# Crocodoctopus/zkstark

Hardware: AMD Instinct MI355X
Metric: field-elements/s through LDE+Merkle+FRI (full STARK-101 prover) (higher is better)
Workload: dtype u32 (mod 3*2^30+1) + SHA-256

## Files before the change

zkstark_amd/csrc/domain.hip:

```cpp
#include <chrono>
#include <cstdarg>
#include <cstdio>
#include <new>

#include "internal.hpp"

namespace zk {
namespace impl {

namespace {
thread_local std::string g_last_error;
}

int fail(int code, const char* fmt, ...) {
    char buf[512];
    va_list ap;
    va_start(ap, fmt);
    vsnprintf(buf, sizeof buf, fmt, ap);
    va_end(ap);
    g_last_error = buf;
    return code;
}
const char* last_error() { return g_last_error.c_str(); }

Plan make_plan(uint32_t log_m) {
    Plan p;
    uint32_t np = (log_m + kMaxRadixLog - 1) / kMaxRadixLog;
    if (np == 0) np = 1;
    uint32_t base = log_m / np, extra = log_m % np;
    p.nd = np;
    for (uint32_t d = 0; d < np; ++d) p.bits[d] = base + (d < extra ? 1 : 0);
    return p;
}

uint32_t pick_logC(uint32_t log_total, uint32_t logR) {
    uint32_t cols = log_total - logR, cap = ntt_pass_tile_log(log_total, logR) - logR;
    return cols < cap ? cols : cap;
}

int build_table(uint32_t root, uint32_t log_order, DevTable* t) {
    uint32_t lo_bits = (log_order + 1) / 2, hi_bits = log_order - lo_bits;
    std::vector<uint32_t> lo((size_t)1 << lo_bits), hi((size_t)1 << hi_bits);
    uint32_t acc = 1;
    for (size_t j = 0; j < lo.size(); ++j) { lo[j] = to_mont(acc); acc = mulmod(acc, root); }
    uint32_t step = powmod(root, (uint64_t)1 << lo_bits);
    acc = 1;
    for (size_t j = 0; j < hi.size(); ++j) { hi[j] = to_mont(acc); acc = mulmod(acc, step); }
    HIPCHK(hipMalloc(&t->lo, lo.size() * 4));
    HIPCHK(hipMalloc(&t->hi, hi.size() * 4));
    HIPCHK(hipMemcpy(t->lo, lo.data(), lo.size() * 4, hipMemcpyHostToDevice));
    HIPCHK(hipMemcpy(t->hi, hi.data(), hi.size() * 4, hipMemcpyHostToDevice));
    t->lo_bits = lo_bits;
    return ZK_OK;
}
void free_table(DevTable* t) {
    if (t->lo) (void)hipFree(t->lo);
    if (t->hi) (void)hipFree(t->hi);
    t->lo = t->hi = nullptr;
}

int run_dif(const uint32_t* src, uint32_t* data, uint32_t log_m, const Plan& pl, PowTable tw_inv, uint32_t L, uint32_t scale_mont, hipStream_t s, Profiler* prof,
            uint32_t batch, size_t src_stride, size_t data_stride) {
    uint32_t inner = log_m;
    for (uint32_t d = 0; d < pl.nd; ++d) {
        inner -= pl.bits[d];
        NttPassArgs a{};
        a.batch = batch; a.src_stride = d == 0 ? src_stride : data_stride; a.dst_stride = data_stride;
        a.src = d == 0 ? src : data; a.dst = data; a.log_total = log_m;
        a.logR = pl.bits[d]; a.logS = inner; a.logC = pick_logC(log_m, a.logR); a.tile_log = ntt_pass_tile_log(log_m, a.logR);
        a.L = L; a.tw = tw_inv; a.scale_mont = (inner == 0) ? scale_mont : 0;
        HIPCHK(launch_ntt_pass(a, NTT_DIF, s, prof));
    }
    return ZK_OK;
}
int run_dit(uint32_t* data, uint32_t log_m, const Plan& pl, PowTable tw, uint32_t L, hipStream_t s) {
    uint32_t inner = 0;
    for (int d = (int)pl.nd - 1; d >= 0; --d) {
        NttPassArgs a{};
        a.src = data; a.dst = data; a.log_total = log_m;
        a.logR = pl.bits[d]; a.logS = inner; a.logC = pick_logC(log_m, a.logR); a.tile_log = ntt_pass_tile_log(log_m, a.logR);
        a.L = L; a.tw = tw;
        HIPCHK(launch_ntt_pass(a, NTT_DIT, s));
        inner += pl.bits[d];
    }
    return ZK_OK;
}



void dom_free(zk_dom* d) {
    if (!d) return;
    free_table(&d->H); free_table(&d->Hinv); free_table(&d->W);
    if (d->d_inv_xm1) (void)hipFree(d->d_inv_xm1);
    delete d;
}

int dom_make(int device, uint32_t log_n, uint32_t log_b, uint32_t shift, bool fold_only, hipStream_t stream, zk_dom** out) {
    *out = nullptr;
    if (log_n < 1 || log_b > 5 || log_n + log_b > 30 || log_n + log_b < 1)
        return fail(ZK_ERR_INVALID, "domain: need 1 <= log_n, log_blowup <= 5, log_n + log_blowup <= 30 (got %u, %u)", log_n, log_b);
    if (shift == 0 || shift >= P) return fail(ZK_ERR_INVALID, "domain: shift must be a non-zero canonical residue");
    HIPCHK(hipSetDevice(device));
    zk_dom* d = new (std::nothrow) zk_dom();
    if (!d) return fail(ZK_ERR_NOMEM, "out of host memory");
    d->device = device;
    d->log_n = log_n; d->log_b = log_b; d->L = log_n + log_b;
    d->n = (size_t)1 << log_n; d->B = (size_t)1 << log_b; d->N = d->n << log_b;
    d->shift = shift;
    d->g = root_of_unity(log_n);
    d->h = root_of_unity(d->L);
    d->plan = make_plan(log_n);
    int rc;
    if ((rc = build_table(d->h, d->L, &d->H)) || (rc = build_table(invmod(d->h), d->L, &d->Hinv))) { dom_free(d); return rc; }
    uint32_t gm1 = invmod(d->g);
    d->shift_mont = to_mont(shift);
    d->gm1_mont = to_mont(gm1);
    d->gm2_mont = to_mont(mulmod(gm1, gm1));
    d->gm3_mont = to_mont(mulmod(mulmod(gm1, gm1), gm1));
    d->ninv_mont = to_mont(invmod((uint32_t)(d->n % P)));
    d->inv2_mont = to_mont(invmod(2));
    {
        const uint32_t inv2 = invmod(2);
        uint32_t wr = shift;
        for (uint32_t r = 0; r < d->L && r < 32; ++r) { d->fold_k[r] = mulmod(invmod(wr), inv2); wr = mulmod(wr, wr); }
        uint32_t xn = powmod(shift, d->n);
        const uint32_t hn = powmod(d->h, d->n);
        for (size_t r = 0; r < d->B; ++r) { const uint32_t den = sub(xn, 1); d->inv_den[r] = den ? invmod(den) : 0u; xn = mulmod(xn, hn); }
    }
    if (!fold_only) {
        if ((rc = build_table(shift, log_n, &d->W))) { dom_free(d); return rc; }
        if (powmod(shift, d->N) == 1) { dom_free(d); return fail(ZK_ERR_INVALID, "domain: shift lies in the evaluation subgroup"); }
        hipError_t e = hipMalloc((void**)&d->d_inv_xm1, d->N * 4);
        if (e != hipSuccess) { dom_free(d); return fail(ZK_ERR_NOMEM, "hipMalloc(%zu) failed", d->N * 4); }
        d->device_bytes += d->N * 4;
        e = launch_build_inv_xm1(d->d_inv_xm1, d->L, d->H.view(), d->shift_mont, stream);
        if (e == hipSuccess) e = hipStreamSynchronize(stream);
        if (e != hipSuccess) { dom_free(d); return fail(ZK_ERR_HIP, "inv_xm1 build failed: %s", hipGetErrorString(e)); }
    }
    *out = d;
    return ZK_OK;
}

int dom_lde(const zk_dom* d, const uint32_t* d_trace, uint32_t* d_coef, uint32_t* d_out, hipStream_t s, Profiler* prof, uint32_t batch) {
    const size_t ts = batch > 1 ? d->n : 0, cs = batch > 1 ? 2 * d->n : 0, os = batch > 1 ? d->N : 0;
    int rc = run_dif(d_trace, d_coef, d->log_n, d->plan, d->Hinv.view(), d->L, 0, s, prof, batch, ts, cs);
    if (rc) return rc;
    uint32_t* d_prep = d_coef + d->n;
    CoefPrepArgs pa{};
    pa.log_n = d->log_n; pa.log_b = d->log_b;
    pa.tw = d->H.view(); pa.wtab = d->W.view(); pa.ninv_mont = d->ninv_mont;
    pa.nd = d->plan.nd;
    for (uint32_t t = 0; t < d->plan.nd; ++t) pa.dig_bits[t] = d->plan.bits[t];
    uint32_t inner = d->log_b;
    for (int q = (int)d->plan.nd - 1; q >= 0; --q) {
        NttPassArgs a{};
        a.log_total = d->L; a.logR = d->plan.bits[q]; a.logS = inner; a.logC = pick_logC(d->L, a.logR); a.tile_log = ntt_pass_tile_log(d->L, a.logR);
        a.L = d->L; a.tw = d->H.view();
        a.dst = d_out;
        a.batch = batch; a.dst_stride = os; a.src_stride = os;
        if (q == (int)d->plan.nd - 1) {
            if (a.logC < d->log_b) a.logC = d->log_b;
            a.src_stride = cs;
            const bool fuse = ntt_fast_ok(a, NTT_DIT_LDE);
            if (fuse) {
                a.src = d_coef;
                a.prep = 1; a.prep_log_n = d->log_n; a.prep_log_b = d->log_b; a.prep_ninv_mont = d->ninv_mont;
                a.prep_nd = d->plan.nd; a.prep_wtab = d->W.view();
                for (uint32_t t = 0; t < d->plan.nd; ++t) a.prep_bits[t] = d->plan.bits[t];
            } else {
                HIPCHK(launch_coef_prepare(d_coef, d_prep, pa, s, prof, batch, cs, cs));
                a.src = d_prep;
            }
            HIPCHK(launch_ntt_pass(a, NTT_DIT_LDE, s, prof));
        } else {
            a.src = d_out;
            HIPCHK(launch_ntt_pass(a, NTT_DIT, s, prof));
        }
        inner += d->plan.bits[q];
    }
    return ZK_OK;
}

int compose_args(const zk_dom* d, const uint32_t* d_f, uint32_t* d_cp, uint32_t first, uint32_t last,
                 const uint32_t alpha_raw[3], ComposeArgs& a) {
    a = ComposeArgs{};
    a.f = d_f; a.inv_xm1 = d->d_inv_xm1; a.cp = d_cp;
    a.logN = d->L; a.log_b = d->log_b;
    a.htab = d->H.view();
    a.w_mont = d->shift_mont; a.gm1_mont = d->gm1_mont; a.gm2_mont = d->gm2_mont; a.gm3_mont = d->gm3_mont;
    a.first = first % P; a.last = last % P;
    uint32_t a0 = alpha_raw[0] % P, a1 = alpha_raw[1] % P, a2 = alpha_raw[2] % P;
    a.alpha0_mont = to_mont(a0);
    a.alpha1g2_mont = to_mont(mulmod(a1, mulmod(d->g, d->g)));
    for (size_t r = 0; r < d->B; ++r) {
        if (d->inv_den[r] == 0) return fail(ZK_ERR_INVALID, "compose: x^n = 1 on the domain");
        a.zz[r] = to_mont(to_mont(mulmod(a2, d->inv_den[r])));
    }
    return ZK_OK;
}
int dom_compose(const zk_dom* d, const uint32_t* d_f, uint32_t* d_cp, uint32_t first, uint32_t last,
                const uint32_t alpha_raw[3], hipStream_t s, Profiler* prof) {
    ComposeArgs a;
    int rc = compose_args(d, d_f, d_cp, first, last, alpha_raw, a);
    if (rc) return rc;
    HIPCHK(launch_compose(a, s, prof));
    return ZK_OK;
}

int fold_args(const zk_dom* d, const uint32_t* d_in, uint32_t* d_out, uint32_t log_m, uint32_t round, uint32_t beta_raw, FoldArgs& a) {
    if (log_m < 1 || log_m + round != d->L) return fail(ZK_ERR_INVALID, "fold: layer size 2^%u does not match round %u of a 2^%u domain", log_m, round, d->L);
    a = FoldArgs{};
    a.in = d_in; a.out = d_out; a.log_m = log_m; a.round = round;
    a.hinv = d->Hinv.view(); a.L = d->L;
    a.inv2_mont = d->inv2_mont;
    a.c_mont = to_mont(mulmod(beta_raw % P, d->fold_k[round]));
    return ZK_OK;
}
int dom_fold(const zk_dom* d, const uint32_t* d_in, uint32_t* d_out, uint32_t log_m, uint32_t round, uint32_t beta_raw,
             hipStream_t s, Profiler* prof) {
    FoldArgs a;
    int rc = fold_args(d, d_in, d_out, log_m, round, beta_raw, a);
    if (rc) return rc;
    HIPCHK(launch_fri_fold(a, s, prof));
    return ZK_OK;
}

int fold_multi_args(const zk_dom* d, const uint32_t* d_in, uint32_t* d_out, uint32_t log_m, uint32_t round, uint32_t steps, uint32_t beta_raw,
                    FoldMultiArgs& a) {
    if (steps < 1 || steps > 3) return fail(ZK_ERR_INVALID, "fold: steps must be 1..3 (got %u)", steps);
    if (log_m < steps || log_m + round != d->L)
        return fail(ZK_ERR_INVALID, "fold: layer size 2^%u does not match round %u + %u steps of a 2^%u domain", log_m, round, steps, d->L);
    a = FoldMultiArgs{};
    a.in = d_in; a.out = d_out; a.log_m = log_m; a.round = round; a.steps = steps;
    a.hinv = d->Hinv.view();
    a.scale_mont = to_mont(invmod(1u << steps));
    const uint32_t S = 1u << steps;
    const uint32_t om_inv = invmod(powmod(d->h, (uint64_t)d->N >> steps));
    uint32_t bk = beta_raw % P, ok = om_inv;
    for (uint32_t k = 0; k < steps; ++k) {
        const uint32_t base = mulmod(bk, mulmod(d->fold_k[round + k], 2));
        uint32_t tw = 1;
        for (uint32_t t = 0; t < (S >> (k + 1)); ++t) { a.c_mont[S - (S >> k) + t] = to_mont(mulmod(base, tw)); tw = mulmod(tw, ok); }
        bk = mulmod(bk, bk); ok = mulmod(ok, ok);
    }
    return ZK_OK;
}
int fold_multi_batch_args(const zk_dom* d, const uint32_t* d_in, uint32_t* d_out, uint32_t log_m, uint32_t round, uint32_t steps,
                          const uint32_t* d_beta_raw, uint32_t beta_stride, uint32_t* d_work, uint32_t batch, FoldMultiBatchArgs& a) {
    a = FoldMultiBatchArgs{};
    if (int rc = fold_multi_args(d, d_in, d_out, log_m, round, steps, 1u, a.a)) return rc;
    if (batch < 1 || ((uint64_t)batch << log_m) > ((uint64_t)1 << 32))
        return fail(ZK_ERR_INVALID, "fold: a batch of %u layers of 2^%u values does not fit 2^32 values", batch, log_m);
    a.beta_raw = d_beta_raw; a.beta_stride = beta_stride; a.cb = d_work; a.batch = batch;
    return ZK_OK;
}
int dom_fold_multi_batch(const zk_dom* d, const uint32_t* d_in, uint32_t* d_out, uint32_t log_m, uint32_t round, uint32_t steps,
                         const uint32_t* d_beta_raw, uint32_t beta_stride, uint32_t* d_work, uint32_t batch, hipStream_t s, Profiler* prof) {
    FoldMultiBatchArgs a;
    int rc = fold_multi_batch_args(d, d_in, d_out, log_m, round, steps, d_beta_raw, beta_stride, d_work, batch, a);
    if (rc) return rc;
    HIPCHK(launch_fri_fold_multi_batch(a, s, prof));
    return ZK_OK;
}
int dom_fold_multi(const zk_dom* d, const uint32_t* d_in, uint32_t* d_out, uint32_t log_m, uint32_t round, uint32_t steps, uint32_t beta_raw,
                   hipStream_t s, Profiler* prof) {
    if (steps == 1) return dom_fold(d, d_in, d_out, log_m, round, beta_raw, s, prof);
    FoldMultiArgs a;
    int rc = fold_multi_args(d, d_in, d_out, log_m, round, steps, beta_raw, a);
    if (rc) return rc;
    HIPCHK(launch_fri_fold_multi(a, s, prof));
    return ZK_OK;
}


int wait_flag(const uint32_t* flag, uint32_t want, hipStream_t stream, int (*poll)(void*), void* poll_user, double timeout_s) {
    auto t0 = std::chrono::steady_clock::now();
// ... 37 lines not shown
```

zkstark_amd/csrc/internal.hpp:

```cpp
#pragma once
#include <hip/hip_runtime.h>

#include <cstddef>
#include <cstring>
#include <string>
#include <vector>

#include "../../include/zkstark_amd.h"
#include "field.hpp"
#include "kernels.hpp"
#include "transcript.hpp"

struct zk_channel {
    zk::Channel ch;
};

namespace zk {
namespace impl {

int fail(int code, const char* fmt, ...);
const char* last_error();

#define HIPCHK(expr)                                                                          \
    do {                                                                                      \
// ... 9 lines not shown
template <> struct AbiMin<zk_shard_stats>     { static constexpr uint32_t v = 112;  static constexpr const char* name = "zk_shard_stats"; };
template <> struct AbiMin<zk_shard_plan_info> { static constexpr uint32_t v = 200;  static constexpr const char* name = "zk_shard_plan_info"; };
template <> struct AbiMin<zk_chain_probe>     { static constexpr uint32_t v = 48;   static constexpr const char* name = "zk_chain_probe"; };
template <class T> inline size_t abi_bytes(const T* p, const char* who) {
    static_assert(sizeof(T) >= AbiMin<T>::v && offsetof(T, struct_size) == 0, "a struct of the C ABI shrank or lost its size field");
    const uint32_t n = p->struct_size;
    if (n < AbiMin<T>::v || n > (1u << 16) || (n > AbiMin<T>::v && n < sizeof(T))) {
        fail(ZK_ERR_INVALID, "%s: %s.struct_size is %u; the caller sets it to sizeof(%s) before the call (ZK_STRUCT_INIT): at least %u bytes "
                             "(ABI version 6), %zu in this library (ABI version %u) -- was the caller compiled against another zkstark_amd.h?",
             who, AbiMin<T>::name, n, AbiMin<T>::name, AbiMin<T>::v, sizeof(T), (unsigned)ZK_ABI_VERSION);
        return 0;
    }
    return n < sizeof(T) ? n : sizeof(T);
}
template <class T> inline int abi_put(T* out, const T& src, const char* who) {
    const size_t k = abi_bytes(out, who);
    if (!k) return ZK_ERR_INVALID;
    memcpy(reinterpret_cast<char*>(out) + sizeof(uint32_t), reinterpret_cast<const char*>(&src) + sizeof(uint32_t), k - sizeof(uint32_t));
    return ZK_OK;
}
template <class T> inline int abi_get(const T* in, T* local, const char* who) {
    const size_t k = abi_bytes(in, who);
    if (!k) return ZK_ERR_INVALID;
    memset(static_cast<void*>(local), 0, sizeof(T));
    memcpy(static_cast<void*>(local), in, k);
    local->struct_size = (uint32_t)sizeof(T);
    return ZK_OK;
}

constexpr uint32_t kMaxQueries = 64;
constexpr uint32_t kHostTopSingle = 8;
constexpr uint32_t kMaxHostLog = 10;
constexpr size_t kMailValsOff = kMailDigests + ((size_t)8 << kMaxHostLog);
constexpr size_t kMailWords = kMailValsOff + ((size_t)2 << kMaxHostLog);
constexpr uint32_t kMaxRadixLog = 8;

inline int check_proof_size(const char* who, uint32_t log_n, uint32_t log_b, uint32_t log_extra = 0) {
    if (log_n < 2 || log_b < 1 || log_b > 5 || log_n + log_b + log_extra > 30)
        return fail(ZK_ERR_INVALID, "%s: need 2 <= log_n, 1 <= log_blowup <= 5, log_n + log_blowup%s <= 30 (got %u, %u)", who,
                    log_extra ? " + log_batch" : "", log_n, log_b);
    if (log_n == 3)
        return fail(ZK_ERR_INVALID, "%s: n = 8 is degenerate for the Fibonacci-square constraints (the degree asserts of prover.rs:156/:169 would fail)", who);
    return ZK_OK;
}

struct Plan {
    uint32_t nd = 0;
    uint32_t bits[kMaxDigits] = {0};
};
Plan make_plan(uint32_t log_m);
uint32_t pick_logC(uint32_t log_total, uint32_t logR);

struct DevTable {
    uint32_t* lo = nullptr;
    uint32_t* hi = nullptr;
    uint32_t lo_bits = 0;
    PowTable view() const { return PowTable{lo, hi, lo_bits}; }
};
int build_table(uint32_t root, uint32_t log_order, DevTable* t);
void free_table(DevTable* t);

int run_dif(const uint32_t* src, uint32_t* data, uint32_t log_m, const Plan& pl, PowTable tw_inv, uint32_t L, uint32_t scale_mont,
            hipStream_t s, Profiler* prof = nullptr, uint32_t batch = 1, size_t src_stride = 0, size_t data_stride = 0);
int run_dit(uint32_t* data, uint32_t log_m, const Plan& pl, PowTable tw, uint32_t L, hipStream_t s);

constexpr uint32_t kGrindHostMaxBits = 10;
struct Grinder;
int grinder_create(int device, void* stream, uint32_t max_jobs, Grinder** out);
void grinder_destroy(Grinder* g);
int grind_device(Grinder* g, const uint8_t* states, size_t count, uint32_t bits, uint64_t start, uint64_t* nonces_out);
int grind_host(const uint8_t state[32], uint32_t bits, uint64_t start, uint32_t threads, uint64_t* nonce_out);
int grind_channel(Grinder* g, Channel& ch, uint32_t bits, uint64_t* nonce_out);

}
}

struct zk_dom {
    int device = 0;
    uint32_t log_n = 0, log_b = 0, L = 0;
    size_t n = 0, N = 0, B = 0;
    uint32_t shift = 0, g = 0, h = 0;
    zk::impl::DevTable H, Hinv, W;
    uint32_t* d_inv_xm1 = nullptr;
    zk::impl::Plan plan;
    uint32_t shift_mont = 0, gm1_mont = 0, gm2_mont = 0, gm3_mont = 0, ninv_mont = 0, inv2_mont = 0;
    uint32_t fold_k[32] = {0};
    uint32_t inv_den[32] = {0};
    size_t device_bytes = 0;
};

namespace zk {
namespace impl {

void dom_free(zk_dom* d);
int dom_make(int device, uint32_t log_n, uint32_t log_b, uint32_t shift, bool fold_only, hipStream_t stream, zk_dom** out);
int dom_lde(const zk_dom* d, const uint32_t* d_trace, uint32_t* d_coef, uint32_t* d_out, hipStream_t s, Profiler* prof, uint32_t batch = 1);
int compose_args(const zk_dom* d, const uint32_t* d_f, uint32_t* d_cp, uint32_t first, uint32_t last, const uint32_t alpha_raw[3], ComposeArgs& a);
int dom_compose(const zk_dom* d, const uint32_t* d_f, uint32_t* d_cp, uint32_t first, uint32_t last, const uint32_t alpha_raw[3],
                hipStream_t s, Profiler* prof);
int fold_args(const zk_dom* d, const uint32_t* d_in, uint32_t* d_out, uint32_t log_m, uint32_t round, uint32_t beta_raw, FoldArgs& a);
int dom_fold(const zk_dom* d, const uint32_t* d_in, uint32_t* d_out, uint32_t log_m, uint32_t round, uint32_t beta_raw, hipStream_t s,
             Profiler* prof);
int fold_multi_args(const zk_dom* d, const uint32_t* d_in, uint32_t* d_out, uint32_t log_m, uint32_t round, uint32_t steps, uint32_t beta_raw,
                    FoldMultiArgs& a);
int dom_fold_multi(const zk_dom* d, const uint32_t* d_in, uint32_t* d_out, uint32_t log_m, uint32_t round, uint32_t steps, uint32_t beta_raw,
                   hipStream_t s, Profiler* prof = nullptr);
int fold_multi_batch_args(const zk_dom* d, const uint32_t* d_in, uint32_t* d_out, uint32_t log_m, uint32_t round, uint32_t steps,
                          const uint32_t* d_beta_raw, uint32_t beta_stride, uint32_t* d_work, uint32_t batch, FoldMultiBatchArgs& a);
int dom_fold_multi_batch(const zk_dom* d, const uint32_t* d_in, uint32_t* d_out, uint32_t log_m, uint32_t round, uint32_t steps,
                         const uint32_t* d_beta_raw, uint32_t beta_stride, uint32_t* d_work, uint32_t batch, hipStream_t s,
                         Profiler* prof = nullptr);

int wait_flag(const uint32_t* flag, uint32_t want, hipStream_t stream, int (*poll)(void*) = nullptr, void* poll_user = nullptr, double timeout_s = 30.0);
double now_us();
int tail_open_begin(zk_ctx* tail, size_t x);
int tail_open_end(zk_ctx* tail, uint32_t* vals_out, uint8_t* paths_out);
void path_nodes(size_t m, size_t leaf, std::vector<size_t>& out);
int merkle_nodes_to_host(int device, hipStream_t s, const uint32_t* d_heap, size_t first, size_t count, uint8_t* out);

}
}
```

zkstark_amd/csrc/kernels.hip:

```cpp
#include "kernels.hpp"

#include <cstdlib>

#include "field.hpp"
#include "fieldhash_f64.hpp"
#include "sha256_quad.hpp"
#include "sha256.hpp"

namespace zk {

__device__ __forceinline__ uint32_t pow_lookup(const PowTable& t, uint32_t e) {
    return mont_mul(t.hi[e >> t.lo_bits], t.lo[e & ((1u << t.lo_bits) - 1u)]);
}

constexpr uint32_t R2_MONT = R2;

__device__ uint32_t mont_inv(uint32_t a) {
    uint32_t r = R1, b = a;
    uint32_t e = P - 2;
#pragma unroll 1
    for (int i = 0; i < 32; ++i) {
        if (e & 1) r = mont_mul(r, b);
        b = mont_mul(b, b);
        e >>= 1;
// ... 29 lines not shown
    const uint32_t col0 = blockIdx.x << logC;
    const uint32_t tile_elems = R << logC;
    const uint32_t tw_shift = p.L - logR - logS;
    const uint32_t smask = (1u << logS) - 1u;

    for (uint32_t j = tid; j < (R >> 1); j += kNttThreads) twl[j] = pow_lookup(p.tw, j << (p.L - logR));

    if (MODE == NTT_DIT_LDE) {
        const uint32_t logB = logS;
        const uint32_t a0 = col0 >> logB;
        for (uint32_t u = tid; u < (tile_elems >> logB); u += kNttThreads) {
            uint32_t ao = u >> logR, t = u & (R - 1u);
            uint32_t v = p.src[((size_t)(a0 + ao) << logR) | t];
            uint32_t row = __brev(t) >> (32u - logR);
            uint32_t* dstp = &tile[row * pitch + (ao << logB)];
            dstp[0] = v;
            for (uint32_t s = 1; s <= smask; ++s) dstp[s] = mont_mul(v, pow_lookup(p.tw, (t * s) << tw_shift));
        }
    } else {
        for (uint32_t l = tid; l < tile_elems; l += kNttThreads) {
            uint32_t t, c;
            tile_coords(l, logR, logS, logC, t, c);
            uint32_t col = col0 + c, a = col >> logS, s = col & smask;
            size_t addr = ((size_t)a << (logR + logS)) | ((size_t)t << logS) | s;
            uint32_t v = p.src[addr];
            uint32_t row = t;
            if (MODE == NTT_DIT) {
                if (logS) v = mont_mul(v, pow_lookup(p.tw, (t * s) << tw_shift));
                row = __brev(t) >> (32u - logR);
            }
            tile[row * pitch + c] = v;
        }
    }
    __syncthreads();

    const uint32_t nb = tile_elems >> 1;
    if (MODE == NTT_DIF) {
        for (int ll = (int)logR - 1; ll >= 0; --ll) {
            for (uint32_t b = tid; b < nb; b += kNttThreads) {
                uint32_t c = b & (C - 1u), pi = b >> logC;
                uint32_t j = pi & ((1u << ll) - 1u);
                uint32_t i = ((pi >> ll) << (ll + 1)) | j;
                uint32_t* x0 = &tile[i * pitch + c];
                uint32_t* x1 = x0 + (pitch << ll);
                uint32_t u = *x0, v = *x1;
                *x0 = add(u, v);
                *x1 = mont_mul(sub(u, v), twl[j << (logR - 1u - ll)]);
            }
            __syncthreads();
        }
    } else {
        for (uint32_t ll = 0; ll < logR; ++ll) {
            for (uint32_t b = tid; b < nb; b += kNttThreads) {
                uint32_t c = b & (C - 1u), pi = b >> logC;
                uint32_t j = pi & ((1u << ll) - 1u);
                uint32_t i = ((pi >> ll) << (ll + 1)) | j;
                uint32_t* x0 = &tile[i * pitch + c];
                uint32_t* x1 = x0 + (pitch << ll);
                uint32_t u = *x0, v = mont_mul(*x1, twl[j << (logR - 1u - ll)]);
                *x0 = add(u, v);
                *x1 = sub(u, v);
            }
            __syncthreads();
        }
    }

    for (uint32_t l = tid; l < tile_elems; l += kNttThreads) {
        uint32_t t, c;
        tile_coords(l, logR, logS, logC, t, c);
        uint32_t col = col0 + c, a = col >> logS, s = col & smask;
        size_t addr = ((size_t)a << (logR + logS)) | ((size_t)t << logS) | s;
        uint32_t v;
        if (MODE == NTT_DIF) {
            v = tile[(__brev(t) >> (32u - logR)) * pitch + c];
            if (logS) v = mont_mul(v, pow_lookup(p.tw, (t * s) << tw_shift));
            else if (p.scale_mont) v = mont_mul(v, p.scale_mont);
        } else {
            v = tile[t * pitch + c];
        }
        p.dst[addr] = v;
    }
}

bool launch_ntt_pass_fast(const NttPassArgs& a, NttMode mode, hipStream_t s, hipError_t* err);

hipError_t launch_ntt_pass(const NttPassArgs& a, NttMode mode, hipStream_t s, Profiler* prof) {
    double bytes = mode == NTT_DIT_LDE ? 4.0 * ((double)((size_t)1 << (a.log_total - a.logS)) + (double)((size_t)1 << a.log_total))
                                       : 8.0 * (double)((size_t)1 << a.log_total);
    const uint32_t batch = a.batch ? a.batch : 1;
    ScopedKernelTimer tm(prof, K_NTT, bytes * batch, s, kNttOpsPerElement * (double)((size_t)1 << a.log_total) * batch * (double)a.logR / 7.0);
    hipError_t ferr = hipSuccess;
    if (launch_ntt_pass_fast(a, mode, s, &ferr)) return ferr;
    uint32_t cols_log = a.log_total - a.logR;
    uint32_t blocks = 1u << (cols_log - a.logC);
    size_t shmem = ((size_t)(1u << a.logR) * ((1u << a.logC) + 1u) + (1u << a.logR) / 2u) * sizeof(uint32_t);
    switch (mode) {
        case NTT_DIF: hipLaunchKernelGGL(ntt_pass_kernel<NTT_DIF>, dim3(blocks, batch), dim3(kNttThreads), shmem, s, a); break;
        case NTT_DIT: hipLaunchKernelGGL(ntt_pass_kernel<NTT_DIT>, dim3(blocks, batch), dim3(kNttThreads), shmem, s, a); break;
        case NTT_DIT_LDE: hipLaunchKernelGGL(ntt_pass_kernel<NTT_DIT_LDE>, dim3(blocks, batch), dim3(kNttThreads), shmem, s, a); break;
    }
    return hipGetLastError();
}

__global__ __launch_bounds__(256) void coef_prepare_kernel(const uint32_t* U, uint32_t* out, CoefPrepArgs a, size_t u_stride, size_t out_stride) {
    const uint32_t pos = blockIdx.x * blockDim.x + threadIdx.x, n = 1u << a.log_n;
    if (pos >= n) return;
    U += (size_t)blockIdx.y * u_stride;
    out += (size_t)blockIdx.y * out_stride;
    uint32_t k = 0, rem = a.log_n, sh = 0;
    for (uint32_t d = 0; d < a.nd; ++d) {
        rem -= a.dig_bits[d];
        k |= ((pos >> rem) & ((1u << a.dig_bits[d]) - 1u)) << sh;
        sh += a.dig_bits[d];
    }
    const uint32_t c_top = U[n - 1u];
    uint32_t v = sub(U[pos], mont_mul(c_top, pow_lookup(a.tw, ((k + 1u) & (n - 1u)) << a.log_b)));
    out[pos] = mont_mul(v, mont_mul(pow_lookup(a.wtab, k), a.ninv_mont));
}

hipError_t launch_coef_prepare(const uint32_t* U, uint32_t* out, const CoefPrepArgs& a, hipStream_t s, Profiler* prof,
                               uint32_t batch, size_t u_stride, size_t out_stride) {
    uint32_t n = 1u << a.log_n;
    ScopedKernelTimer tm(prof, K_NTT, 8.0 * n * batch, s);
    hipLaunchKernelGGL(coef_prepare_kernel, dim3((n + 255) / 256, batch), dim3(256), 0, s, U, out, a, u_stride, out_stride);
    return hipGetLastError();
}

struct DigitArgs {
    uint32_t nd;
    uint32_t bits[kMaxDigits];
};

__global__ void digit_reverse_kernel(const uint32_t* in, uint32_t* out, uint32_t log_m, DigitArgs dg, int to_natural) {
    size_t pos = (size_t)blockIdx.x * blockDim.x + threadIdx.x;
    if (pos >= ((size_t)1 << log_m)) return;
    uint32_t k = 0, rem = log_m, sh = 0;
    for (uint32_t d = 0; d < dg.nd; ++d) {
        rem -= dg.bits[d];
        k |= (((uint32_t)pos >> rem) & ((1u << dg.bits[d]) - 1u)) << sh;
        sh += dg.bits[d];
    }
    if (to_natural) out[k] = in[pos];
    else out[pos] = in[k];
}

hipError_t launch_digit_reverse(const uint32_t* in, uint32_t* out, uint32_t log_m, uint32_t nd,
                                const uint32_t* dig_bits, int to_natural, hipStream_t s) {
    DigitArgs dg{};
    dg.nd = nd;
    for (uint32_t i = 0; i < nd; ++i) dg.bits[i] = dig_bits[i];
    size_t m = (size_t)1 << log_m;
    uint32_t threads = 256, blocks = (uint32_t)((m + threads - 1) / threads);
    hipLaunchKernelGGL(digit_reverse_kernel, dim3(blocks), dim3(threads), 0, s, in, out, log_m, dg, to_natural);
    return hipGetLastError();
}

__global__ void degree_check_kernel(const uint32_t* coef, uint32_t log_m, DigitArgs dg, uint32_t bound, uint32_t* out) {
    size_t pos = (size_t)blockIdx.x * blockDim.x + threadIdx.x;
    if (pos >= ((size_t)1 << log_m)) return;
    uint32_t k = 0, rem = log_m, sh = 0;
    for (uint32_t d = 0; d < dg.nd; ++d) {
        rem -= dg.bits[d];
        k |= (((uint32_t)pos >> rem) & ((1u << dg.bits[d]) - 1u)) << sh;
        sh += dg.bits[d];
    }
    const uint32_t v = coef[pos];
    if (k >= bound && v != 0) atomicAdd(&out[0], 1u);
    if (k + 1 == bound) out[1] = v;
}
hipError_t launch_degree_check(const uint32_t* coef, uint32_t log_m, uint32_t nd, const uint32_t* dig_bits, uint32_t bound, uint32_t* out, hipStream_t s) {
    DigitArgs dg{};
    dg.nd = nd;
    for (uint32_t i = 0; i < nd; ++i) dg.bits[i] = dig_bits[i];
    size_t m = (size_t)1 << log_m;
    hipLaunchKernelGGL(degree_check_kernel, dim3((uint32_t)((m + 255) / 256)), dim3(256), 0, s, coef, log_m, dg, bound, out);
    return hipGetLastError();
}


constexpr int kInvBatch = 8;

__global__ __launch_bounds__(256) void build_inv_xm1_kernel(uint32_t* out, size_t count, uint32_t e0, uint32_t order_mask, PowTable htab, uint32_t w_mont) {
    size_t gid = (size_t)blockIdx.x * blockDim.x + threadIdx.x;
    size_t base = gid * kInvBatch;
    if (base >= count) return;
    uint32_t d[kInvBatch], pre[kInvBatch];
    uint32_t acc = R1;
#pragma unroll
    for (int e = 0; e < kInvBatch; ++e) {
        size_t i = base + e;
        uint32_t x = i < count ? mont_mul(pow_lookup(htab, (e0 + (uint32_t)i) & order_mask), w_mont) : add(R1, R1);
        d[e] = sub(x, R1);
        pre[e] = acc;
        acc = mont_mul(acc, d[e]);
    }
    uint32_t inv = mont_inv(acc);
#pragma unroll
    for (int e = kInvBatch - 1; e >= 0; --e) {
        size_t i = base + e;
        uint32_t r = mont_mul(inv, pre[e]);
        inv = mont_mul(inv, d[e]);
        if (i < count) out[i] = r;
    }
}

hipError_t launch_build_inv_xm1_range(uint32_t* out, size_t count, uint32_t e0, uint32_t log_order, PowTable htab, uint32_t shift_mont, hipStream_t s) {
    size_t threads_total = (count + kInvBatch - 1) / kInvBatch;
    uint32_t blocks = (uint32_t)((threads_total + 255) / 256);
    if (!blocks) return hipSuccess;
    hipLaunchKernelGGL(build_inv_xm1_kernel, dim3(blocks), dim3(256), 0, s, out, count, e0, (uint32_t)(((uint64_t)1 << log_order) - 1u), htab, shift_mont);
    return hipGetLastError();
}
hipError_t launch_build_inv_xm1(uint32_t* out, uint32_t logN, PowTable htab, uint32_t shift_mont, hipStream_t s) {
    return launch_build_inv_xm1_range(out, (size_t)1 << logN, 0u, logN, htab, shift_mont, s);
}

struct ComposeRaw { uint32_t f0, f1, f2, inv0, inv2, x_hi, x_lo, zz; };
__device__ __forceinline__ ComposeRaw compose_fetch(const ComposeArgs& a, const uint32_t* f, size_t i) {
    const size_t N = (size_t)1 << a.logN;
    const uint32_t B = 1u << a.log_b;
    const size_t i1 = (i + B) & (N - 1), i2 = (i + 2 * (size_t)B) & (N - 1);
    ComposeRaw r;
    r.f0 = f[i]; r.f1 = f[i1]; r.f2 = f[i2];
    r.inv0 = a.inv_xm1[i]; r.inv2 = a.inv_xm1[i2];
    r.x_hi = a.htab.hi[(uint32_t)i >> a.htab.lo_bits]; r.x_lo = a.htab.lo[(uint32_t)i & ((1u << a.htab.lo_bits) - 1u)];
    r.zz = a.zz[i & (B - 1)];
    return r;
}
template <bool BATCH>
__device__ __forceinline__ uint32_t compose_eval(const ComposeArgs& a, uint32_t f0, uint32_t f1, uint32_t f2, uint32_t inv0, uint32_t inv2,
                                                 uint32_t x, uint32_t zz, uint32_t first, uint32_t last, uint32_t al0, uint32_t al1g2, uint32_t al2) {
    uint32_t t0 = mont_mul(mont_mul(sub(f0, first), inv0), al0);
    uint32_t t1 = mont_mul(mont_mul(sub(f0, last), inv2), al1g2);
    uint32_t v3 = mont_mul(mont_mul(sub(x, a.gm3_mont), sub(x, a.gm2_mont)), sub(x, a.gm1_mont));
    uint32_t y = mont_mul(v3, zz);
    if (BATCH) y = mont_mul(y, al2);
    uint32_t num = sub(sub(mont_mul(f2, 1u), mont_mul(f1, f1)), mont_mul(f0, f0));
    uint32_t t2 = mont_mul(num, y);
    return add(add(t0, t1), t2);
}
template <bool BATCH>
__device__ __forceinline__ uint32_t compose_finish(const ComposeArgs& a, const ComposeRaw& r, uint32_t first, uint32_t last, uint32_t al0,
                                                   uint32_t al1g2, uint32_t al2) {
    const uint32_t x = mont_mul(mont_mul(r.x_hi, r.x_lo), a.w_mont);
    return compose_eval<BATCH>(a, r.f0, r.f1, r.f2, r.inv0, r.inv2, x, r.zz, first, last, al0, al1g2, al2);
}
template <bool BATCH>
__device__ __forceinline__ uint32_t compose_core(const ComposeArgs& a, const uint32_t* f, uint32_t first, uint32_t last, uint32_t al0,
                                                 uint32_t al1g2, uint32_t al2, size_t i) {
    return compose_finish<BATCH>(a, compose_fetch(a, f, i), first, last, al0, al1g2, al2);
}
__device__ __forceinline__ uint32_t compose_at(const ComposeArgs& a, size_t i) {
    return compose_core<false>(a, a.f, a.first, a.last, a.alpha0_mont, a.alpha1g2_mont, 0u, i);
}

__global__ __launch_bounds__(256) void compose_kernel(ComposeArgs a) {
    size_t i = (size_t)blockIdx.x * blockDim.x + threadIdx.x;
    if (i >= ((size_t)1 << a.logN)) return;
    a.cp[i] = compose_at(a, i);
}

__global__ __launch_bounds__(256) void compose_kernel4(ComposeArgs a) {
    const size_t N = (size_t)1 << a.logN;
    const uint32_t B = 1u << a.log_b;
    const size_t i = ((size_t)blockIdx.x * blockDim.x + threadIdx.x) * 4;
    if (i >= N) return;
    const uint4* fv = reinterpret_cast<const uint4*>(a.f);
    const uint4* iv = reinterpret_cast<const uint4*>(a.inv_xm1);
    uint32_t f0[4], f1[4], f2[4], inv0[4], inv2[4], zz[4];
    const uint4 v0 = fv[i >> 2], w0 = iv[i >> 2];
    f0[0] = v0.x; f0[1] = v0.y; f0[2] = v0.z; f0[3] = v0.w;
    inv0[0] = w0.x; inv0[1] = w0.y; inv0[2] = w0.z; inv0[3] = w0.w;
    if (B >= 4) {
        const uint4 v1 = fv[((i + B) & (N - 1)) >> 2], v2 = fv[((i + 2 * (size_t)B) & (N - 1)) >> 2], w2 = iv[((i + 2 * (size_t)B) & (N - 1)) >> 2];
        f1[0] = v1.x; f1[1] = v1.y; f1[2] = v1.z; f1[3] = v1.w;
        f2[0] = v2.x; f2[1] = v2.y; f2[2] = v2.z; f2[3] = v2.w;
        inv2[0] = w2.x; inv2[1] = w2.y; inv2[2] = w2.z; inv2[3] = w2.w;
        const uint32_t z0 = (uint32_t)i & (B - 1);
#pragma unroll
        for (int k = 0; k < 4; ++k) zz[k] = a.zz[z0 + k];
    } else {
        const uint4 v1 = fv[((i + 4) & (N - 1)) >> 2], w1 = iv[((i + 4) & (N - 1)) >> 2];
        const uint32_t fw[8] = {v0.x, v0.y, v0.z, v0.w, v1.x, v1.y, v1.z, v1.w};
        const uint32_t iw[8] = {w0.x, w0.y, w0.z, w0.w, w1.x, w1.y, w1.z, w1.w};
#pragma unroll
        for (int k = 0; k < 4; ++k) {
            f1[k] = B == 1 ? fw[k + 1] : fw[k + 2];
            f2[k] = B == 1 ? fw[k + 2] : fw[k + 4];
            inv2[k] = B == 1 ? iw[k + 2] : iw[k + 4];
            zz[k] = B == 1 ? a.zz[0] : a.zz[k & 1];
        }
    }
    uint32_t x = mont_mul(pow_lookup(a.htab, (uint32_t)i), a.w_mont);
    const uint32_t h = pow_lookup(a.htab, 1u);
    uint32_t r[4];
#pragma unroll
    for (int k = 0; k < 4; ++k) {
        r[k] = compose_eval<false>(a, f0[k], f1[k], f2[k], inv0[k], inv2[k], x, zz[k], a.first, a.last, a.alpha0_mont, a.alpha1g2_mont, 0u);
        if (k < 3) x = mont_mul(x, h);
    }
    reinterpret_cast<uint4*>(a.cp)[i >> 2] = make_uint4(r[0], r[1], r[2], r[3]);
}

hipError_t launch_compose(const ComposeArgs& a, hipStream_t s, Profiler* prof) {
    size_t N = (size_t)1 << a.logN;
    ScopedKernelTimer tm(prof, K_COMPOSE, 8.0 * (double)N, s);
    const bool aligned = ((reinterpret_cast<uintptr_t>(a.f) | reinterpret_cast<uintptr_t>(a.inv_xm1) | reinterpret_cast<uintptr_t>(a.cp)) & 15u) == 0;
    if (a.logN >= 4 && aligned) {
        uint32_t blocks = (uint32_t)((N / 4 + 255) / 256);
        hipLaunchKernelGGL(compose_kernel4, dim3(blocks), dim3(256), 0, s, a);
    } else {
        uint32_t blocks = (uint32_t)((N + 255) / 256);
        hipLaunchKernelGGL(compose_kernel, dim3(blocks), dim3(256), 0, s, a);
    }
    return hipGetLastError();
}

struct FoldRaw { uint32_t u, v, x_hi, x_lo; };
__device__ __forceinline__ FoldRaw fold_fetch(const FoldArgs& a, size_t i) {
    const size_t half = (size_t)1 << (a.log_m - 1);
    const uint32_t e = (uint32_t)(i << a.round);
    FoldRaw r;
    r.u = a.in[i]; r.v = a.in[i + half];
    r.x_hi = a.hinv.hi[e >> a.hinv.lo_bits]; r.x_lo = a.hinv.lo[e & ((1u << a.hinv.lo_bits) - 1u)];
    return r;
}
__device__ __forceinline__ uint32_t fold_finish(const FoldArgs& a, const FoldRaw& r) {
    uint32_t xinv = mont_mul(r.x_hi, r.x_lo);
    uint32_t s = mont_mul(add(r.u, r.v), a.inv2_mont);
    uint32_t d = mont_mul(mont_mul(sub(r.u, r.v), xinv), a.c_mont);
    return add(s, d);
}
__device__ __forceinline__ uint32_t fold_at(const FoldArgs& a, size_t i) { return fold_finish(a, fold_fetch(a, i)); }

__global__ __launch_bounds__(256) void fri_fold_kernel(FoldArgs a) {
    size_t i = (size_t)blockIdx.x * blockDim.x + threadIdx.x;
    if (i >= ((size_t)1 << (a.log_m - 1))) return;
    a.out[i] = fold_at(a, i);
}

__global__ __launch_bounds__(256) void fri_fold_kernel4(FoldArgs a) {
    const size_t half = (size_t)1 << (a.log_m - 1);
    const size_t i = ((size_t)blockIdx.x * blockDim.x + threadIdx.x) * 4;
    if (i >= half) return;
    const uint4 u = reinterpret_cast<const uint4*>(a.in)[i >> 2], v = reinterpret_cast<const uint4*>(a.in)[(i + half) >> 2];
    const uint32_t uu[4] = {u.x, u.y, u.z, u.w}, vv[4] = {v.x, v.y, v.z, v.w};
    uint32_t xinv = pow_lookup(a.hinv, (uint32_t)(i << a.round));
    const uint32_t step = pow_lookup(a.hinv, 1u << a.round);
    uint32_t r[4];
#pragma unroll
    for (int k = 0; k < 4; ++k) {
        const uint32_t sm = mont_mul(add(uu[k], vv[k]), a.inv2_mont);
        const uint32_t d = mont_mul(mont_mul(sub(uu[k], vv[k]), xinv), a.c_mont);
        r[k] = add(sm, d);
        if (k < 3) xinv = mont_mul(xinv, step);
    }
    reinterpret_cast<uint4*>(a.out)[i >> 2] = make_uint4(r[0], r[1], r[2], r[3]);
}

hipError_t launch_fri_fold(const FoldArgs& a, hipStream_t s, Profiler* prof) {
    size_t half = (size_t)1 << (a.log_m - 1);
    ScopedKernelTimer tm(prof, K_FOLD, 12.0 * (double)half, s);
    const bool aligned = ((reinterpret_cast<uintptr_t>(a.in) | reinterpret_cast<uintptr_t>(a.out)) & 15u) == 0;
    if (half >= 4 && aligned) {
        uint32_t blocks = (uint32_t)((half / 4 + 255) / 256);
        hipLaunchKernelGGL(fri_fold_kernel4, dim3(blocks), dim3(256), 0, s, a);
    } else {
        uint32_t blocks = (uint32_t)((half + 255) / 256);
        hipLaunchKernelGGL(fri_fold_kernel, dim3(blocks), dim3(256), 0, s, a);
    }
    return hipGetLastError();
}

template <int STEPS>
__device__ __forceinline__ uint32_t fold_multi_core(const uint32_t (&c)[7], uint32_t scale_mont, uint32_t (&v)[1 << STEPS], uint32_t xinv) {
    constexpr int S = 1 << STEPS;
#pragma unroll
    for (int k = 0; k < STEPS; ++k) {
        const int cnt = S >> (k + 1);
#pragma unroll
        for (int t = 0; t < cnt; ++t) {
            const uint32_t u = v[t], w = v[t + cnt];
            v[t] = add(add(u, w), mont_mul(sub(u, w), mont_mul(xinv, c[S - (S >> k) + t])));
        }
        if (k + 1 < STEPS) xinv = mont_mul(xinv, xinv);
    }
    return mont_mul(v[0], scale_mont);
}
template <int STEPS>
__device__ __forceinline__ uint32_t fold_multi_one(const FoldMultiArgs& a, uint32_t (&v)[1 << STEPS], uint32_t xinv) {
    return fold_multi_core<STEPS>(a.c_mont, a.scale_mont, v, xinv);
}

template <int STEPS>
__global__ __launch_bounds__(256) void fri_fold_multi_kernel1(FoldMultiArgs a) {
    constexpr int S = 1 << STEPS;
    const size_t q = (size_t)1 << (a.log_m - STEPS);
    const size_t i = (size_t)blockIdx.x * blockDim.x + threadIdx.x;
    if (i >= q) return;
    uint32_t v[S];
#pragma unroll
    for (int t = 0; t < S; ++t) v[t] = a.in[i + t * q];
    a.out[i] = fold_multi_one<STEPS>(a, v, pow_lookup(a.hinv, (uint32_t)(i << a.round)));
}

template <int STEPS>
__global__ __launch_bounds__(256) void fri_fold_multi_kernel(FoldMultiArgs a) {
    constexpr int S = 1 << STEPS;
    const size_t q = (size_t)1 << (a.log_m - STEPS);
    const size_t i = ((size_t)blockIdx.x * blockDim.x + threadIdx.x) * 4;
    if (i >= q) return;
    uint4 ld[S];
#pragma unroll
    for (int t = 0; t < S; ++t) ld[t] = reinterpret_cast<const uint4*>(a.in)[(i + t * q) >> 2];
    uint32_t xinv = pow_lookup(a.hinv, (uint32_t)(i << a.round));
    const uint32_t step = pow_lookup(a.hinv, 1u << a.round);
    uint32_t r[4];
#pragma unroll
    for (int e = 0; e < 4; ++e) {
        uint32_t v[S];
#pragma unroll
        for (int t = 0; t < S; ++t) v[t] = e == 0 ? ld[t].x : e == 1 ? ld[t].y : e == 2 ? ld[t].z : ld[t].w;
        r[e] = fold_multi_one<STEPS>(a, v, xinv);
        if (e < 3) xinv = mont_mul(xinv, step);
    }
    reinterpret_cast<uint4*>(a.out)[i >> 2] = make_uint4(r[0], r[1], r[2], r[3]);
}

template <int STEPS>
static void fold_multi_launch(const FoldMultiArgs& a, size_t q, bool wide, hipStream_t s) {
    if (wide) hipLaunchKernelGGL(fri_fold_multi_kernel<STEPS>, dim3((uint32_t)((q / 4 + 255) / 256)), dim3(256), 0, s, a);
    else hipLaunchKernelGGL(fri_fold_multi_kernel1<STEPS>, dim3((uint32_t)((q + 255) / 256)), dim3(256), 0, s, a);
}
hipError_t launch_fri_fold_multi(const FoldMultiArgs& a, hipStream_t s, Profiler* prof) {
    if (a.steps < 1 || a.steps > 3 || a.log_m < a.steps) return hipErrorInvalidValue;
    const size_t m = (size_t)1 << a.log_m, q = m >> a.steps;
    ScopedKernelTimer tm(prof, K_FOLD, 4.0 * (double)(m + q), s);
    const bool wide = q >= 4 && ((reinterpret_cast<uintptr_t>(a.in) | reinterpret_cast<uintptr_t>(a.out)) & 15u) == 0;
    if (a.steps == 1) fold_multi_launch<1>(a, q, wide, s);
    else if (a.steps == 2) fold_multi_launch<2>(a, q, wide, s);
    else fold_multi_launch<3>(a, q, wide, s);
    return hipGetLastError();
}

template <int STEPS>
__global__ __launch_bounds__(256) void fri_fold_multi_batch_prep_kernel(FoldMultiBatchArgs p) {
    constexpr int S = 1 << STEPS;
    const uint32_t b = blockIdx.x * blockDim.x + threadIdx.x;
    if (b >= p.batch) return;
    uint32_t bk = mont_mul(p.beta_raw[(size_t)b * p.beta_stride], R2_MONT);
    uint32_t c[8] = {0, 0, 0, 0, 0, 0, 0, 0};
#pragma unroll
    for (int k = 0; k < STEPS; ++k) {
#pragma unroll
        for (int t = 0; t < (S >> (k + 1)); ++t) c[S - (S >> k) + t] = mont_mul(bk, p.a.c_mont[S - (S >> k) + t]);
        if (k + 1 < STEPS) bk = mont_mul(bk, bk);
    }
    uint32_t* row = p.cb + (size_t)b * 8;
#pragma unroll
    for (int j = 0; j < 8; ++j) row[j] = c[j];
}
template <int STEPS>
__device__ __forceinline__ void fold_multi_batch_consts(const FoldMultiBatchArgs& p, size_t b, uint32_t (&c)[7]) {
    constexpr int S = 1 << STEPS;
    const uint32_t* row = p.cb + b * 8;
#pragma unroll
    for (int j = 0; j < 7; ++j) c[j] = j < S - 1 ? row[j] : 0u;
}

template <int STEPS>
__global__ __launch_bounds__(256) void fri_fold_multi_batch_kernel1(FoldMultiBatchArgs p) {
    constexpr int S = 1 << STEPS;
    const uint32_t log_q = p.a.log_m - STEPS;
    const size_t q = (size_t)1 << log_q;
    const size_t pos = (size_t)blockIdx.x * blockDim.x + threadIdx.x;
    if (pos >= ((size_t)p.batch << log_q)) return;
    const size_t b = pos >> log_q, i = pos & (q - 1);
    const uint32_t* in = p.a.in + (b << p.a.log_m);
    uint32_t v[S];
#pragma unroll
    for (int t = 0; t < S; ++t) v[t] = in[i + t * q];
    uint32_t c[7];
    fold_multi_batch_consts<STEPS>(p, b, c);
    p.a.out[pos] = fold_multi_core<STEPS>(c, p.a.scale_mont, v, pow_lookup(p.a.hinv, (uint32_t)(i << p.a.round)));
}

template <int STEPS>
__global__ __launch_bounds__(256) void fri_fold_multi_batch_kernel(FoldMultiBatchArgs p) {
    constexpr int S = 1 << STEPS;
    const uint32_t log_q = p.a.log_m - STEPS;
    const size_t q = (size_t)1 << log_q;
    const size_t pos = ((size_t)blockIdx.x * blockDim.x + threadIdx.x) * 4;
    if (pos >= ((size_t)p.batch << log_q)) return;
    const size_t b = pos >> log_q, i = pos & (q - 1);
    const uint32_t* in = p.a.in + (b << p.a.log_m);
    uint4 ld[S];
#pragma unroll
    for (int t = 0; t < S; ++t) ld[t] = reinterpret_cast<const uint4*>(in)[(i + t * q) >> 2];
    uint32_t c[7];
    fold_multi_batch_consts<STEPS>(p, b, c);
    uint32_t xinv = pow_lookup(p.a.hinv, (uint32_t)(i << p.a.round));
    const uint32_t step = pow_lookup(p.a.hinv, 1u << p.a.round);
    uint32_t r[4];
#pragma unroll
    for (int e = 0; e < 4; ++e) {
        uint32_t v[S];
#pragma unroll
        for (int t = 0; t < S; ++t) v[t] = e == 0 ? ld[t].x : e == 1 ? ld[t].y : e == 2 ? ld[t].z : ld[t].w;
        r[e] = fold_multi_core<STEPS>(c, p.a.scale_mont, v, xinv);
        if (e < 3) xinv = mont_mul(xinv, step);
    }
    reinterpret_cast<uint4*>(p.a.out)[pos >> 2] = make_uint4(r[0], r[1], r[2], r[3]);
}

template <int STEPS>
static void fold_multi_batch_launch(const FoldMultiBatchArgs& p, size_t total, bool wide, hipStream_t s) {
    hipLaunchKernelGGL(fri_fold_multi_batch_prep_kernel<STEPS>, dim3((p.batch + 255) / 256), dim3(256), 0, s, p);
    if (wide) hipLaunchKernelGGL(fri_fold_multi_batch_kernel<STEPS>, dim3((uint32_t)((total / 4 + 255) / 256)), dim3(256), 0, s, p);
    else hipLaunchKernelGGL(fri_fold_multi_batch_kernel1<STEPS>, dim3((uint32_t)((total + 255) / 256)), dim3(256), 0, s, p);
}
hipError_t launch_fri_fold_multi_batch(const FoldMultiBatchArgs& p, hipStream_t s, Profiler* prof) {
    const FoldMultiArgs& a = p.a;
    if (a.steps < 1 || a.steps > 3 || a.log_m < a.steps || a.log_m > 32 || p.batch < 1 || !p.beta_raw || !p.cb) return hipErrorInvalidValue;
    const size_t m = (size_t)1 << a.log_m, q = m >> a.steps, total = (size_t)p.batch * q;
    if ((size_t)p.batch * m > ((size_t)1 << 32)) return hipErrorInvalidValue;
    ScopedKernelTimer tm(prof, K_FOLD, 4.0 * (double)p.batch * (double)(m + q), s);
    const bool wide = q >= 4 && ((reinterpret_cast<uintptr_t>(a.in) | reinterpret_cast<uintptr_t>(a.out)) & 15u) == 0;
    if (a.steps == 1) fold_multi_batch_launch<1>(p, total, wide, s);
    else if (a.steps == 2) fold_multi_batch_launch<2>(p, total, wide, s);
    else fold_multi_batch_launch<3>(p, total, wide, s);
    return hipGetLastError();
}


__constant__ FieldHashConsts g_fh_consts;
__constant__ FieldHashConsts64 g_fh_consts64;

template <int HASH> struct Hasher;
template <> struct Hasher<0> {
    static __device__ __forceinline__ Digest leaf(uint32_t v) { return sha256_leaf(v); }
    static __device__ __forceinline__ Digest inner(const Digest& l, const Digest& r) { return sha256_inner(l, r); }
};
template <> struct Hasher<1> {
    static __device__ __forceinline__ Digest leaf(uint32_t v) { return fieldhash_leaf64(v, g_fh_consts64); }
    static __device__ __forceinline__ Digest inner(const Digest& l, const Digest& r) { return fieldhash_inner64(l, r, g_fh_consts64); }
};

struct PlainSrc {
    const uint32_t* vals;
    using Raw = uint32_t;
    __device__ __forceinline__ Raw fetch(size_t pos) const { return vals[pos]; }
    __device__ __forceinline__ uint32_t finish(const Raw& r, size_t) const { return r; }
    __device__ __forceinline__ uint32_t load(size_t pos) const { return vals[pos]; }
};
struct FoldSrc {
    FoldArgs a;
    using Raw = FoldRaw;
    __device__ __forceinline__ void prepare() { if (a.dyn) a.c_mont = *a.dyn; }
    __device__ __forceinline__ Raw fetch(size_t pos) const { return fold_fetch(a, pos); }
    __device__ __forceinline__ uint32_t finish(const Raw& r, size_t pos) const { uint32_t v = fold_finish(a, r); a.out[pos] = v; return v; }
    __device__ __forceinline__ uint32_t load(size_t pos) const { return finish(fetch(pos), pos); }
};
struct ComposeSrc {
    ComposeArgs a;
    using Raw = size_t;
    __device__ __forceinline__ Raw fetch(size_t pos) const { return pos; }
    __device__ __forceinline__ uint32_t finish(const Raw& r, size_t) const { return load(r); }
    __device__ __forceinline__ uint32_t load(size_t pos) const { uint32_t v = compose_at(a, pos); a.cp[pos] = v; return v; }
};

struct ComposeBlockSrc {
    ComposeBlockArgs b;
    using Raw = size_t;
    __device__ __forceinline__ uint32_t f_at(size_t t) const {
        const uint32_t gmask = (1u << b.lg) - 1u;
        if (t >> b.log_m) {
            const size_t v = t - ((size_t)1 << b.log_m);
            return b.halo[(v & gmask) * b.halo_stride + (v >> b.lg)];
        }
        const uint32_t log_cl = b.lg + b.log_cnt;
        const size_t piece = ((t >> log_cl) << b.lg) | (t & gmask);
        return b.a.f[(piece << b.log_cnt) | ((t & (((size_t)1 << log_cl) - 1)) >> b.lg)];
    }
    __device__ __forceinline__ Raw fetch(size_t pos) const { return pos; }
    __device__ __forceinline__ uint32_t finish(const Raw& r, size_t) const { return load(r); }
    __device__ __forceinline__ uint32_t load(size_t pos) const {
        const ComposeArgs& a = b.a;
        const size_t B = (size_t)1 << a.log_b;
        const uint32_t f0 = f_at(pos), f1 = f_at(pos + B), f2 = f_at(pos + 2 * B);
        const uint32_t x = mont_mul(pow_lookup(a.htab, b.e0 + (uint32_t)pos), a.w_mont);
        return compose_eval<false>(a, f0, f1, f2, a.inv_xm1[pos], a.inv_xm1[pos + 2 * B], x, a.zz[pos & (B - 1)], a.first, a.last, a.alpha0_mont,
                                   a.alpha1g2_mont, 0u);
    }
};

struct ComposeBatchSrc {
    ComposeArgs a;
    const BatchChal* chal;
    using Raw = size_t;
    __device__ __forceinline__ Raw fetch(size_t pos) const { return pos; }
    __device__ __forceinline__ uint32_t finish(const Raw& r, size_t) const { return load(r); }
    __device__ __forceinline__ uint32_t load(size_t pos) const {
        const size_t b = pos >> a.logN, i = pos & (((size_t)1 << a.logN) - 1);
        const BatchChal c = chal[b];
        uint32_t v = compose_core<true>(a, a.f + (b << a.logN), c.first, c.last, c.alpha0_mont, c.alpha1g2_mont, c.alpha2_mont, i);
        a.cp[pos] = v;
        return v;
    }
};
struct FoldBatchSrc {
    FoldArgs a;
    const BatchChal* chal;
    using Raw = size_t;
    __device__ __forceinline__ Raw fetch(size_t pos) const { return pos; }
    __device__ __forceinline__ uint32_t finish(const Raw& r, size_t) const { return load(r); }
    __device__ __forceinline__ uint32_t load(size_t pos) const {
        const uint32_t lh = a.log_m - 1;
        const size_t half = (size_t)1 << lh, b = pos >> lh, i = pos & (half - 1);
        const uint32_t* in = a.in + (b << a.log_m);
        uint32_t u = in[i], v = in[i + half];
        uint32_t xinv = pow_lookup(a.hinv, (uint32_t)(i << a.round));
        uint32_t s = mont_mul(add(u, v), a.inv2_mont);
        uint32_t d = mont_mul(mont_mul(sub(u, v), xinv), chal[b].c_mont);
        uint32_t r = add(s, d);
        a.out[pos] = r;
        return r;
    }
};

struct InterleaveSrc {
    const uint32_t* recv;
    uint32_t log_parts, log_cnt;
    using Raw = uint32_t;
    __device__ __forceinline__ uint32_t load(size_t pos) const {
        return recv[((pos & (((size_t)1 << log_parts) - 1)) << log_cnt) | (pos >> log_parts)];
    }
    __device__ __forceinline__ Raw fetch(size_t pos) const { return load(pos); }
    __device__ __forceinline__ uint32_t finish(const Raw& r, size_t) const { return r; }
};

template <class S> __device__ __forceinline__ auto src_prepare(S& s, int) -> decltype(s.prepare(), void()) { s.prepare(); }
template <class S> __device__ __forceinline__ void src_prepare(S&, long) {}

constexpr int kMerkleThreads = 256;
constexpr uint32_t kMerkleMaxK = 4;

__device__ __forceinline__ void store_digest(uint32_t* nodes, size_t node, const Digest& d) {
    uint4* q = reinterpret_cast<uint4*>(nodes + node * 8);
    q[0] = make_uint4(d.w[0], d.w[1], d.w[2], d.w[3]);
    q[1] = make_uint4(d.w[4], d.w[5], d.w[6], d.w[7]);
}
__device__ __forceinline__ Digest load_digest(const uint32_t* nodes, size_t node) {
    const uint4* q = reinterpret_cast<const uint4*>(nodes + node * 8);
    uint4 lo = q[0], hi = q[1];
    Digest d;
    d.w[0] = lo.x; d.w[1] = lo.y; d.w[2] = lo.z; d.w[3] = lo.w;
    d.w[4] = hi.x; d.w[5] = hi.y; d.w[6] = hi.z; d.w[7] = hi.w;
    return d;
}

__device__ __forceinline__ Digest lds_digest(const uint4* p) {
    uint4 lo = p[0], hi = p[1];
    Digest d;
    d.w[0] = lo.x; d.w[1] = lo.y; d.w[2] = lo.z; d.w[3] = lo.w;
    d.w[4] = hi.x; d.w[5] = hi.y; d.w[6] = hi.z; d.w[7] = hi.w;
    return d;
}

template <class SRC, bool LEAF, int HASH>
__global__ __launch_bounds__(kMerkleThreads) void merkle_subtree_kernel(SRC src, uint32_t* nodes,
                                                                        uint32_t depth_in, uint32_t k, size_t off) {
    extern __shared__ __attribute__((aligned(16))) uint4 stage[];
    src_prepare(src, 0);
    const uint32_t lane = threadIdx.x & 63u, wave = threadIdx.x >> 6;
    const size_t gwave = (size_t)blockIdx.x * (kMerkleThreads / 64) + wave;
    const size_t base = (gwave << (6 + k)) + off;
    const size_t in_base = ((size_t)1 << depth_in) - 1;
    uint4* my = stage + (size_t)wave * (k + 1) * 128;
    uint4* scratch = my + (size_t)k * 128;
    typename SRC::Raw raw;
    Digest dnext;
    uint32_t val = 0;
    if (LEAF) val = src.load(base + lane - off);
    else dnext = load_digest(nodes, in_base + base + lane);
#pragma unroll 1
    for (uint32_t i = 0; i < (1u << k); ++i) {
        Digest d;
        const size_t pos = base + (size_t)i * 64 + lane;
        const bool more = i + 1 < (1u << k);
        if (LEAF) {
            if (more) raw = src.fetch(pos + 64 - off);
            d = Hasher<HASH>::leaf(val);
            store_digest(nodes, in_base + pos, d);
        } else {
            d = dnext;
            if (more) dnext = load_digest(nodes, in_base + pos + 64);
        }
        uint32_t idx = i, lvl = 0;
#pragma unroll 1
        while (lvl < k) {
            uint4* left = my + lvl * 128;
            uint4* grp = (idx & 1u) ? scratch : left;
            grp[2 * lane] = make_uint4(d.w[0], d.w[1], d.w[2], d.w[3]);
            grp[2 * lane + 1] = make_uint4(d.w[4], d.w[5], d.w[6], d.w[7]);
            if (!(idx & 1u)) break;
// ... 387 lines not shown
    static bool done[64] = {false};
    int dev = 0;
    hipError_t e = hipGetDevice(&dev);
    if (e != hipSuccess) return e;
    if (dev < 0 || dev >= 64 || done[dev]) return hipSuccess;
    FieldHashConsts c;
    fieldhash_make_consts(c);
    e = hipMemcpyToSymbol(HIP_SYMBOL(g_fh_consts), &c, sizeof c);
    if (e != hipSuccess) return e;
    static FieldHashConsts64 c64;
    fieldhash_make_consts64(c, c64);
    e = hipMemcpyToSymbol(HIP_SYMBOL(g_fh_consts64), &c64, sizeof c64);
    if (e == hipSuccess) done[dev] = true;
    return e;
}

#ifndef ZK_MERKLE_MAX_K
#define ZK_MERKLE_MAX_K 4
#endif
#ifndef ZK_MERKLE_LATENCY_LOG
#define ZK_MERKLE_LATENCY_LOG 17
#endif
#ifndef ZK_MERKLE_CHUNK_K
#define ZK_MERKLE_CHUNK_K 3
#endif
static_assert(ZK_MERKLE_MAX_K >= 1 && ZK_MERKLE_MAX_K <= (int)kMerkleMaxK && ZK_MERKLE_CHUNK_K >= 1 && ZK_MERKLE_CHUNK_K <= (int)kMerkleMaxK, "levels per launch");
static_assert(ZK_MERKLE_LATENCY_LOG >= 12 && ZK_MERKLE_LATENCY_LOG <= 24, "latency switch");
static uint32_t g_merkle_latency_log = ZK_MERKLE_LATENCY_LOG;
static constexpr uint32_t merkle_max_k() { return ZK_MERKLE_MAX_K; }
static uint32_t merkle_latency_log() { return __atomic_load_n(&g_merkle_latency_log, __ATOMIC_RELAXED); }
bool set_merkle_latency_log(uint32_t v) {
    if (v == 0) v = ZK_MERKLE_LATENCY_LOG;
    if (v < 12 || v > 24) return false;
    __atomic_store_n(&g_merkle_latency_log, v, __ATOMIC_RELAXED);
    return true;
}

static double wg_level_us(uint32_t w, int hash) {
    if (w == 0) return 0.0;
    if (hash) return w <= kFieldRowMaxNodes ? (double)((w + 15) / 16) * 3.7 : w <= kFieldQuadMaxNodes ? (double)((w + 63) / 64) * 5.3 : (double)((w + 255) / 256) * 10.8;
    return w <= 64 ? 3.1 : w <= 128 ? 4.9 : (double)((w + 255) / 256) * 4.6;
}
static double wg_phase_us(bool leaf, uint32_t cnt_log, uint32_t levels, int hash, uint32_t blocks) {
    const uint32_t cnt = 1u << cnt_log;
    double us = !leaf ? 1.0
                : hash ? (cnt <= kFieldRowLeafMax ? (double)((cnt + 15) / 16) * 3.7 : (double)((cnt + 255) / 256) * 10.8)
                       : (double)((cnt + 255) / 256) * 2.6;
    for (uint32_t t = 1; t <= levels; ++t) us += wg_level_us(cnt >> t, hash);
    return blocks > 256 ? us * (double)blocks / 256.0 : us;
}
#ifndef ZK_MERKLE_CONTINUATION
#define ZK_MERKLE_CONTINUATION 1
#endif
static constexpr bool g_merkle_continuation = ZK_MERKLE_CONTINUATION != 0;
constexpr double kContinueUs = 6.0;
constexpr double kLaunchUs = 10.0;

template <class SRC>
static hipError_t merkle_build_t(SRC src, double src_bytes, uint32_t log_m, uint32_t* nodes, hipStream_t s, Profiler* prof,
                                 const MailArgs& mail_in, int hash, uint32_t log_sub = 0xffffffffu, size_t chunk = 0,
                                 bool leaf_mode = true, uint32_t tp_floor = 0) {
    if (hash) {
        hipError_t e = ensure_fieldhash_consts();
        if (e != hipSuccess) return e;
    }
    if (log_sub == 0xffffffffu) log_sub = log_m;
    const uint32_t stop = log_m - log_sub;
    uint32_t depth = log_m;
    bool leaf = leaf_mode;
    const PlainSrc none{nullptr};
    auto first_bytes = [&](double b) { return leaf ? b - 4.0 * (double)((size_t)1 << log_sub) + src_bytes : b; };
    const uint32_t kMerkleLatencyLog = merkle_latency_log();
    auto off_at = [&](uint32_t d) { return (size_t)chunk << (d - stop); };
    const bool throughput_only = tp_floor != 0;
    const uint32_t floor_depth = throughput_only ? tp_floor : stop + kMerkleLatencyLog;
    while (depth > floor_depth) {
        uint32_t k = depth - floor_depth;
        if (k > merkle_max_k()) k = merkle_max_k();
        size_t lanes = (size_t)1 << (depth - stop - k);
        uint32_t blocks = (uint32_t)(lanes / kMerkleThreads);
        size_t sh = (size_t)(kMerkleThreads / 64) * (k + 1) * 128 * sizeof(uint4);
        ScopedKernelTimer tm(prof, leaf ? K_MERKLE_LEAF : K_MERKLE_INNER, first_bytes(merkle_bytes(leaf, depth - stop, k)), s, merkle_ops(leaf, depth - stop, k, hash));
        if (hash) {
            if (leaf) hipLaunchKernelGGL((merkle_subtree_kernel<SRC, true, 1>), dim3(blocks), dim3(kMerkleThreads), sh, s, src, nodes, depth, k, off_at(depth));
            else hipLaunchKernelGGL((merkle_subtree_kernel<PlainSrc, false, 1>), dim3(blocks), dim3(kMerkleThreads), sh, s, none, nodes, depth, k, off_at(depth));
        } else {
            if (leaf) hipLaunchKernelGGL((merkle_subtree_kernel<SRC, true, 0>), dim3(blocks), dim3(kMerkleThreads), sh, s, src, nodes, depth, k, off_at(depth));
            else hipLaunchKernelGGL((merkle_subtree_kernel<PlainSrc, false, 0>), dim3(blocks), dim3(kMerkleThreads), sh, s, none, nodes, depth, k, off_at(depth));
        }
        leaf = false;
        depth -= k;
    }
    if (throughput_only) return hipGetLastError();
    MailArgs mail = mail_in;
    if (stop != 0 || mail.top >= log_m) mail.top = 0;
    const uint32_t end = stop == 0 ? mail.top : stop;
    auto launch_wg = [&](uint32_t j, uint32_t j2) {
        const uint32_t span = depth - stop;
        const uint32_t blocks = 1u << (span - j);
        const uint32_t lds_log = j2 && span - j > j ? span - j : j;
        const size_t sh = ((size_t)2 << lds_log) * sizeof(uint4) + 2 * 16 * 128 * sizeof(uint32_t);
        ScopedKernelTimer tm(prof, K_MERKLE_TOP, first_bytes(merkle_bytes(leaf, span, j)) + (j2 ? merkle_bytes(false, span - j, j2) : 0.0), s,
                             merkle_ops(leaf, span, j, hash) + (j2 ? merkle_ops(false, span - j, j2, hash) : 0.0));
        if (hash) {
            if (leaf) hipLaunchKernelGGL((merkle_wg_kernel<SRC, true, 1>), dim3(blocks), dim3(kWgThreads), sh, s, src, nodes, depth, j, mail, off_at(depth), j2, lds_log);
            else hipLaunchKernelGGL((merkle_wg_kernel<PlainSrc, false, 1>), dim3(blocks), dim3(kWgThreads), sh, s, none, nodes, depth, j, mail, off_at(depth), j2, lds_log);
        } else {
            if (leaf) hipLaunchKernelGGL((merkle_wg_kernel<SRC, true, 0>), dim3(blocks), dim3(kWgThreads), sh, s, src, nodes, depth, j, mail, off_at(depth), j2, lds_log);
            else hipLaunchKernelGGL((merkle_wg_kernel<PlainSrc, false, 0>), dim3(blocks), dim3(kWgThreads), sh, s, none, nodes, depth, j, mail, off_at(depth), j2, lds_log);
        }
        leaf = false;
        depth -= j + j2;
    };
    const bool may_continue = stop == 0 && mail.counter != nullptr && g_merkle_continuation;
    do {
        const uint32_t span = depth - stop;
        const uint32_t levels = depth - end;
        const uint32_t launches = levels ? (levels + kWgMaxLog - 1) / kWgMaxLog : 1;
        const uint32_t jn = (levels + launches - 1) / launches;
        uint32_t best_j = jn, best_j2 = 0;
        if (may_continue && levels <= 2 * kWgMaxLog) {
            double best = wg_phase_us(leaf, jn, jn, hash, 1u << (span - jn));
            if (launches == 2 && span - jn <= kWgMaxLog) best += kLaunchUs + wg_phase_us(false, span - jn, levels - jn, hash, 1);
            else if (launches > 1) best = 0.0;
            for (uint32_t j = 1; j < levels && j <= kWgMaxLog; ++j) {
                const uint32_t j2 = levels - j;
                if (j2 > kWgMaxLog || span - j > kWgMaxLog) continue;
                const double us = wg_phase_us(leaf, j, j, hash, 1u << (span - j)) + kContinueUs + wg_phase_us(false, span - j, j2, hash, 1);
                if (us < best) { best = us; best_j = j; best_j2 = j2; }
            }
        }
        launch_wg(best_j, best_j2);
    } while (depth > end);
    return hipGetLastError();
}

hipError_t launch_merkle_build(const uint32_t* vals, uint32_t log_m, uint32_t* nodes, hipStream_t s, Profiler* prof,
                               const MailArgs& mail, int hash) {
    return merkle_build_t(PlainSrc{vals}, 4.0 * (double)((size_t)1 << log_m), log_m, nodes, s, prof, mail, hash);
}
hipError_t launch_merkle_build_interleaved(const uint32_t* recv, uint32_t log_parts, uint32_t log_cnt, uint32_t* nodes, hipStream_t s,
                                           Profiler* prof, int hash, const MailArgs& mail) {
    uint32_t log_m = log_parts + log_cnt;
    return merkle_build_t(InterleaveSrc{recv, log_parts, log_cnt}, 4.0 * (double)((size_t)1 << log_m), log_m, nodes, s, prof, mail, hash);
}
static constexpr uint32_t merkle_chunk_k() { return ZK_MERKLE_CHUNK_K; }
static uint32_t chunk_handover_depth(uint32_t log_m, uint32_t log_chunks) {
    const uint32_t lat = merkle_latency_log();
    if (!(log_m > lat && lat >= log_chunks + 8)) return log_chunks;
    uint32_t k = log_m - lat < merkle_max_k() ? log_m - lat : merkle_max_k();
    if (k > merkle_chunk_k()) k = merkle_chunk_k();
    return log_m - k;
}
uint32_t merkle_finish_start_depth(uint32_t log_m, uint32_t log_chunks) { return chunk_handover_depth(log_m, log_chunks); }
hipError_t launch_merkle_build_chunk(const uint32_t* recv, uint32_t log_parts, uint32_t log_cnt, uint32_t* nodes, uint32_t log_m,
                                     uint32_t chunk, hipStream_t s, Profiler* prof, int hash) {
    uint32_t log_sub = log_parts + log_cnt;
    const uint32_t h = chunk_handover_depth(log_m, log_m - log_sub);
    return merkle_build_t(InterleaveSrc{recv, log_parts, log_cnt}, 4.0 * (double)((size_t)1 << log_sub), log_m, nodes, s, prof, MailArgs{}, hash,
                          log_sub, chunk, true, h != log_m - log_sub ? h : 0u);
}
hipError_t launch_merkle_finish(uint32_t* nodes, uint32_t log_m, uint32_t log_chunks, hipStream_t s, Profiler* prof, int hash,
                                const MailArgs& mail) {
    const uint32_t start = chunk_handover_depth(log_m, log_chunks);
    if (start == 0) return hipSuccess;
    return merkle_build_t(PlainSrc{nullptr}, 0.0, start, nodes, s, prof, mail, hash, start, 0, false);
}
hipError_t launch_fold_merkle(const FoldArgs& a, uint32_t* nodes, hipStream_t s, Profiler* prof, const MailArgs& mail, int hash) {
    uint32_t log_out = a.log_m - 1;
    return merkle_build_t(FoldSrc{a}, 12.0 * (double)((size_t)1 << log_out), log_out, nodes, s, prof, mail, hash);
}
hipError_t launch_compose_merkle(const ComposeArgs& a, uint32_t* nodes, hipStream_t s, Profiler* prof, const MailArgs& mail, int hash) {
    return merkle_build_t(ComposeSrc{a}, 8.0 * (double)((size_t)1 << a.logN), a.logN, nodes, s, prof, mail, hash);
}

hipError_t launch_compose_block_merkle(const ComposeBlockArgs& b, uint32_t* nodes, hipStream_t s, Profiler* prof, const MailArgs& mail, int hash) {
    return merkle_build_t(ComposeBlockSrc{b}, 8.0 * (double)((size_t)1 << b.log_m), b.log_m, nodes, s, prof, mail, hash);
}

hipError_t launch_compose_merkle_batch(const ComposeBatchArgs& a, uint32_t log_batch, uint32_t* nodes, hipStream_t s, Profiler* prof,
                                       const MailArgs& mail, int hash) {
    uint32_t log_m = a.a.logN + log_batch;
    return merkle_build_t(ComposeBatchSrc{a.a, a.chal}, 8.0 * (double)((size_t)1 << log_m), log_m, nodes, s, prof, mail, hash);
}
hipError_t launch_fold_merkle_batch(const FoldBatchArgs& a, uint32_t log_batch, uint32_t* nodes, hipStream_t s, Profiler* prof,
                                    const MailArgs& mail, int hash) {
    uint32_t log_out = a.a.log_m - 1 + log_batch;
    return merkle_build_t(FoldBatchSrc{a.a, a.chal}, 12.0 * (double)((size_t)1 << log_out), log_out, nodes, s, prof, mail, hash);
}

__global__ __launch_bounds__(1024) void scatter_kernel(const uint32_t* stage, const ScatterSeg* segs, uint32_t* trees, uint32_t* layers) {
    const ScatterSeg sg = segs[blockIdx.x];
    uint32_t* dst = (sg.kind ? layers : trees) + sg.dst;
    const uint32_t* src = stage + sg.src;
    if (((sg.src | sg.dst | sg.words) & 3) == 0) {
        const uint4* s4 = reinterpret_cast<const uint4*>(src);
        uint4* d4 = reinterpret_cast<uint4*>(dst);
        for (uint32_t i = threadIdx.x; i < sg.words / 4; i += blockDim.x) d4[i] = s4[i];
    } else {
        for (uint32_t i = threadIdx.x; i < sg.words; i += blockDim.x) dst[i] = src[i];
    }
}
hipError_t launch_scatter(const uint32_t* stage, const ScatterSeg* segs, uint32_t count, double words, uint32_t* trees, uint32_t* layers,
                          hipStream_t s, Profiler* prof) {
    if (!count) return hipSuccess;
    ScopedKernelTimer tm(prof, K_GATHER, 8.0 * words, s);
    hipLaunchKernelGGL(scatter_kernel, dim3(count), dim3(1024), 0, s, stage, segs, trees, layers);
    return hipGetLastError();
}

template <int HASH>
__global__ __launch_bounds__(256) void hash_chain_probe_kernel(uint32_t* out, uint32_t seed, uint32_t hashes, unsigned long long* rec) {
    Digest d;
#pragma unroll
    for (int i = 0; i < 8; ++i) d.w[i] = (seed * (uint32_t)(i + 1) + threadIdx.x + blockIdx.x * 977u) % P;
    const unsigned long long c0 = __builtin_amdgcn_s_memtime(), r0 = __builtin_amdgcn_s_memrealtime();
#pragma unroll 1
    for (uint32_t it = 0; it < hashes; ++it) {
        Digest r = d;
        r.w[0] ^= seed;
        if (HASH) r.w[0] &= 0x7fffffffu;
        d = Hasher<HASH>::inner(d, r);
    }
    const unsigned long long c1 = __builtin_amdgcn_s_memtime(), r1 = __builtin_amdgcn_s_memrealtime();
    uint32_t x = 0;
#pragma unroll
    for (int i = 0; i < 8; ++i) x ^= d.w[i];
    out[blockIdx.x * 256 + threadIdx.x] = x;
    if (rec && (threadIdx.x & 63) == 0) {
        rec[((size_t)blockIdx.x * 4 + (threadIdx.x >> 6)) * 2] = c1 - c0;
        rec[((size_t)blockIdx.x * 4 + (threadIdx.x >> 6)) * 2 + 1] = r1 - r0;
    }
}
hipError_t launch_hash_chain_probe(int hash, uint32_t blocks, uint32_t* out, uint32_t seed, uint32_t hashes, unsigned long long* rec, hipStream_t s) {
    if (hash) {
        hipError_t e = ensure_fieldhash_consts();
        if (e != hipSuccess) return e;
        hipLaunchKernelGGL(hash_chain_probe_kernel<1>, dim3(blocks), dim3(256), 0, s, out, seed, hashes, rec);
    } else {
        hipLaunchKernelGGL(hash_chain_probe_kernel<0>, dim3(blocks), dim3(256), 0, s, out, seed, hashes, rec);
    }
    return hipGetLastError();
}

__global__ __launch_bounds__(256) void fieldhash_forms_kernel(uint32_t seed, uint32_t* bad, uint32_t* first_bad) {
    const uint32_t t = blockIdx.x * blockDim.x + threadIdx.x;
    uint32_t x = (t + 1u) * 2654435761u + seed;
    auto rnd = [&]() { x ^= x << 13; x ^= x >> 17; x ^= x << 5; return x; };
    Digest l, r;
#pragma unroll
    for (int i = 0; i < 8; ++i) { l.w[i] = rnd() % P; r.w[i] = rnd() % P; }
    if ((t & 15u) == 1) { l.w[t & 7u] = 0; r.w[(t >> 4) & 7u] = P - 1; }
    if ((t & 15u) == 2) {
#pragma unroll
        for (int i = 0; i < 8; ++i) { l.w[i] = P - 1; r.w[i] = P - 1; }
    }
    if ((t & 15u) == 3) { l.w[0] = 0xFFFFFFFFu; r.w[7] = P; r.w[3] = P + 5; }
    if ((t & 15u) == 4) {
#pragma unroll
        for (int i = 0; i < 8; ++i) { l.w[i] = 0; r.w[i] = 0; }
    }
    uint32_t v = rnd();
    if ((t & 7u) == 0) v = (t & 8u) ? 0xFFFFFFFFu : P - 1;
    if (t == 5) v = 0;
    const Digest a = fieldhash_inner(l, r, g_fh_consts), b = fieldhash_inner64(l, r, g_fh_consts64);
    const Digest c = fieldhash_leaf(v, g_fh_consts), d = fieldhash_leaf64(v, g_fh_consts64);
    bool ok = true;
#pragma unroll
    for (int i = 0; i < 8; ++i) ok = ok && a.w[i] == b.w[i] && c.w[i] == d.w[i] && b.w[i] < P && d.w[i] < P;
    const uint32_t g = threadIdx.x & 15u;
    uint32_t word = 0;
#pragma unroll
    for (int i = 0; i < 8; ++i) {
        const uint32_t lw = __shfl(l.w[i], (int)(threadIdx.x & ~15u) & 63, 64), rw = __shfl(r.w[i], (int)(threadIdx.x & ~15u) & 63, 64);
        if (g == (uint32_t)i) word = lw;
        if (g == (uint32_t)i + 8u) word = rw;
    }
    {
        const uint32_t q4 = threadIdx.x & 3u;
        const int src = (int)(threadIdx.x & ~3u) & 63;
        uint32_t in4[4], out4[4];
#pragma unroll
        for (int j = 0; j < 4; ++j) {
            uint32_t wsel = 0;
#pragma unroll
            for (int i = 0; i < 8; ++i) {
                const uint32_t lw = __shfl(l.w[i], src, 64), rw = __shfl(r.w[i], src, 64);
                if ((int)(4 * q4) + j == i) wsel = lw;
                if ((int)(4 * q4) + j == i + 8) wsel = rw;
            }
// ... 61 lines not shown
    uint32_t* row = out + (size_t)t * stride;
    uint32_t x = mont_mul(a0[t], R2_MONT), y = mont_mul(a1[t], R2_MONT);
    if (count > 0) row[0] = mont_mul(x, 1u);
    if (count > 1) row[1] = mont_mul(y, 1u);
    for (uint32_t i = 2; i < count; ++i) {
        uint32_t z = add(mont_mul(x, x), mont_mul(y, y));
        row[i] = mont_mul(z, 1u);
        x = y; y = z;
    }
}

hipError_t launch_trace_fibsq_batch(const uint32_t* a0, const uint32_t* a1, uint32_t batch, uint32_t count, uint32_t* out, hipStream_t s,
                                    uint32_t stride) {
    if (!batch) return hipSuccess;
    hipLaunchKernelGGL(trace_fibsq_batch_kernel, dim3((batch + 63) / 64), dim3(64), 0, s, a0, a1, batch, count, out, stride ? stride : count);
    return hipGetLastError();
}

__global__ void interleave_kernel(const uint32_t* in, uint32_t* out, uint32_t log_parts, uint32_t log_cnt) {
    size_t o = (size_t)blockIdx.x * blockDim.x + threadIdx.x;
    if (o >= ((size_t)1 << (log_parts + log_cnt))) return;
    size_t q = o & (((size_t)1 << log_parts) - 1), u = o >> log_parts;
    out[o] = in[(q << log_cnt) + u];
}

__global__ __launch_bounds__(256) void halo_pack_kernel(const uint32_t* loc, uint32_t* out, uint32_t log_per, uint32_t lg, uint32_t h) {
    const uint32_t i = blockIdx.x * blockDim.x + threadIdx.x;
    if (i >= (h << lg)) return;
    const uint32_t q = i / h, u = i - q * h;
    const size_t mask = ((size_t)1 << (log_per + lg)) - 1;
    out[i] = loc[((((size_t)q + 1) << log_per) + u) & mask];
}
hipError_t launch_halo_pack(const uint32_t* loc, uint32_t* out, uint32_t log_per, uint32_t lg, uint32_t h, hipStream_t s) {
    const uint32_t total = h << lg;
    hipLaunchKernelGGL(halo_pack_kernel, dim3((total + 255) / 256), dim3(256), 0, s, loc, out, log_per, lg, h);
    return hipGetLastError();
}
hipError_t launch_interleave(const uint32_t* in, uint32_t* out, uint32_t log_parts, uint32_t log_cnt, hipStream_t s) {
    size_t total = (size_t)1 << (log_parts + log_cnt);
    uint32_t blocks = (uint32_t)((total + 255) / 256);
    hipLaunchKernelGGL(interleave_kernel, dim3(blocks), dim3(256), 0, s, in, out, log_parts, log_cnt);
    return hipGetLastError();
}

__global__ void pattern_fill_kernel(uint32_t* dst, uint32_t rank, uint32_t log_per, uint32_t log_parts) {
    const size_t i = (size_t)blockIdx.x * blockDim.x + threadIdx.x;
    if (i >= ((size_t)1 << (log_per + log_parts))) return;
    dst[i] = shard_pattern(rank, (uint32_t)(i >> log_per), (uint32_t)(i & (((size_t)1 << log_per) - 1)));
}
__global__ void pattern_check_kernel(const uint32_t* src, uint32_t rank, uint32_t log_per, uint32_t log_parts, uint32_t log_chunks, uint32_t* out) {
    const size_t i = (size_t)blockIdx.x * blockDim.x + threadIdx.x;
    if (i >= ((size_t)1 << (log_per + log_parts))) return;
    const uint32_t log_cc = log_per - log_chunks;
    const uint32_t u = (uint32_t)(i & (((size_t)1 << log_cc) - 1));
    const uint32_t q = (uint32_t)(i >> log_cc) & ((1u << log_parts) - 1u), c = (uint32_t)(i >> (log_cc + log_parts));
    if (src[i] != shard_pattern(q, rank, (c << log_cc) | u)) {
        atomicAdd(&out[0], 1u);
        atomicMin(&out[1], (uint32_t)i);
    }
}
hipError_t launch_pattern_fill(uint32_t* dst, uint32_t rank, uint32_t log_per, uint32_t log_parts, hipStream_t s) {
    const size_t total = (size_t)1 << (log_per + log_parts);
    hipLaunchKernelGGL(pattern_fill_kernel, dim3((uint32_t)((total + 255) / 256)), dim3(256), 0, s, dst, rank, log_per, log_parts);
    return hipGetLastError();
}
hipError_t launch_pattern_check(const uint32_t* src, uint32_t rank, uint32_t log_per, uint32_t log_parts, uint32_t log_chunks, uint32_t* out, hipStream_t s) {
    const size_t total = (size_t)1 << (log_per + log_parts);
    hipLaunchKernelGGL(pattern_check_kernel, dim3((uint32_t)((total + 255) / 256)), dim3(256), 0, s, src, rank, log_per, log_parts, log_chunks, out);
    return hipGetLastError();
}

__global__ void gather_kernel(const uint32_t* src, const uint64_t* offsets, uint32_t count, uint32_t words, uint32_t* out) {
    uint32_t idx = blockIdx.x * blockDim.x + threadIdx.x;
    if (idx >= count * words) return;
    uint32_t item = idx / words, w = idx % words;
    out[idx] = src[offsets[item] + w];
}

hipError_t launch_gather(const uint32_t* src, const uint64_t* offsets, uint32_t count, uint32_t words,
                         uint32_t* out, hipStream_t s, Profiler* prof) {
    if (!count) return hipSuccess;
    ScopedKernelTimer tm(prof, K_GATHER, 8.0 * (double)count * words, s);
    uint32_t total = count * words, blocks = (total + 255) / 256;
    hipLaunchKernelGGL(gather_kernel, dim3(blocks), dim3(256), 0, s, src, offsets, count, words, out);
    return hipGetLastError();
}


constexpr int kFetchThreads = 1024;
__global__ __launch_bounds__(kFetchThreads) void fetch_kernel(const uint32_t* layers, const uint32_t* trees, const uint64_t* items, uint32_t nv,
                                                              uint32_t ndg, uint32_t* out, uint32_t* mailbox, uint32_t seq, uint32_t* counter) {
    const uint32_t stride = gridDim.x * kFetchThreads;
    for (uint32_t idx = blockIdx.x * kFetchThreads + threadIdx.x; idx < 2 * ndg + nv; idx += stride) {
        if (idx < 2 * ndg) {
            const uint4* src = reinterpret_cast<const uint4*>(trees + items[nv + (idx >> 1)]);
            reinterpret_cast<uint4*>(out)[idx] = src[idx & 1u];
        } else {
            const uint32_t i = idx - 2 * ndg;
            out[8 * (size_t)ndg + i] = layers[items[i]];
        }
    }
    __threadfence_system();
    __syncthreads();
    if (threadIdx.x == 0) {
        bool last = true;
        if (gridDim.x > 1) {
            last = __hip_atomic_fetch_add(counter, 1u, __ATOMIC_ACQ_REL, __HIP_MEMORY_SCOPE_AGENT) == gridDim.x - 1;
            if (last) __hip_atomic_store(counter, 0u, __ATOMIC_RELAXED, __HIP_MEMORY_SCOPE_AGENT);
        }
        if (last) __hip_atomic_store(&mailbox[0], seq, __ATOMIC_RELEASE, __HIP_MEMORY_SCOPE_SYSTEM);
    }
}

hipError_t launch_fetch(const uint32_t* layers, const uint32_t* trees, const uint64_t* items, uint32_t nv, uint32_t ndg, uint32_t* out,
                        uint32_t* mailbox, uint32_t seq, uint32_t* counter, hipStream_t s, Profiler* prof) {
    ScopedKernelTimer tm(prof, K_GATHER, 8.0 * ((double)nv + 8.0 * (double)ndg), s);
    const uint32_t work = 2 * ndg + nv;
    uint32_t blocks = (work + kFetchThreads - 1) / kFetchThreads;
    if (blocks == 0) blocks = 1;
    if (blocks > 64) blocks = 64;
    hipLaunchKernelGGL(fetch_kernel, dim3(blocks), dim3(kFetchThreads), 0, s, layers, trees, items, nv, ndg, out, mailbox, seq, counter);
    return hipGetLastError();
}

}
```

zkstark_amd/csrc/kernels.hpp:

```cpp
#pragma once
#include <hip/hip_runtime.h>
#include <stddef.h>
#include <stdint.h>

#include <vector>

namespace zk {

enum KernelClass : int {
    K_NTT = 0,
    K_MERKLE_LEAF = 1,
    K_MERKLE_INNER = 2,
    K_MERKLE_TOP = 3,
    K_COMPOSE = 4,
    K_FOLD = 5,
    K_GATHER = 6,
    K_COUNT = 7
};

constexpr double kShaLeafOps = 1259.0;
constexpr double kShaInnerOps = 2293.0;
constexpr double kNttOpsPerElement = 57.0;
constexpr double kFieldLeafOps = 5015.0;
constexpr double kFieldInnerOps = 5072.0;

struct Profiler {
    uint32_t mask = 0;
    struct Rec { int cls; hipEvent_t a, b; double bytes, ops; };
    std::vector<Rec> recs;
    std::vector<hipEvent_t> pool;
    hipEvent_t get() {
        if (!pool.empty()) { hipEvent_t e = pool.back(); pool.pop_back(); return e; }
        hipEvent_t e = nullptr;
        (void)hipEventCreate(&e);
        return e;
    }
    bool on(int cls) const { return (mask >> cls) & 1u; }
};

struct ScopedKernelTimer {
    Profiler* p; int cls; double bytes, ops; hipStream_t s; hipEvent_t a = nullptr;
    ScopedKernelTimer(Profiler* p_, int cls_, double bytes_, hipStream_t s_, double ops_ = 0.0) : p(p_), cls(cls_), bytes(bytes_), ops(ops_), s(s_) {
        if (p && p->on(cls)) { a = p->get(); (void)hipEventRecord(a, s); }
    }
    ~ScopedKernelTimer() {
        if (a) { hipEvent_t b = p->get(); (void)hipEventRecord(b, s); p->recs.push_back({cls, a, b, bytes, ops}); }
    }
};

struct PowTable {
    const uint32_t* lo;
    const uint32_t* hi;
    uint32_t lo_bits;
};

constexpr int kMaxDigits = 6;

enum NttMode : uint32_t {
    NTT_DIF = 0,
    NTT_DIT = 1,
    NTT_DIT_LDE = 2,
};

#ifndef ZK_NTT_SMALL_MAX_LOG
#define ZK_NTT_SMALL_MAX_LOG 20
#endif
constexpr uint32_t kMidTileLog = 12, kSmallTileLog = 11;
constexpr uint32_t kNttSmallTileMaxLog = ZK_NTT_SMALL_MAX_LOG;
inline uint32_t ntt_tile_log(uint32_t log_total) { return log_total <= kNttSmallTileMaxLog ? kSmallTileLog : kMidTileLog; }
inline uint32_t ntt_pass_tile_log(uint32_t log_total, uint32_t logR) {
    const uint32_t t = ntt_tile_log(log_total);
    return logR + 3 > t ? (logR + 3 < kMidTileLog ? logR + 3 : kMidTileLog) : t;
}

struct NttPassArgs {
    const uint32_t* src;
    uint32_t* dst;
    uint32_t log_total;
    uint32_t logR, logS;
    uint32_t logC;
    uint32_t tile_log;
    uint32_t L;
    PowTable tw;
    uint32_t scale_mont;
    uint32_t batch;
    size_t src_stride, dst_stride;
    uint32_t prep;
    uint32_t prep_log_n, prep_log_b, prep_ninv_mont, prep_nd;
    uint32_t prep_bits[kMaxDigits];
    PowTable prep_wtab;
};
bool ntt_fast_ok(const NttPassArgs& a, NttMode mode);

struct CoefPrepArgs {
    uint32_t log_n, log_b;
    PowTable tw;
    PowTable wtab;
    uint32_t ninv_mont;
    uint32_t nd;
    uint32_t dig_bits[kMaxDigits];
};
hipError_t launch_coef_prepare(const uint32_t* U, uint32_t* out, const CoefPrepArgs& a, hipStream_t s, Profiler* prof = nullptr,
                               uint32_t batch = 1, size_t u_stride = 0, size_t out_stride = 0);

hipError_t launch_ntt_pass(const NttPassArgs& a, NttMode mode, hipStream_t s, Profiler* prof = nullptr);
hipError_t launch_digit_reverse(const uint32_t* in, uint32_t* out, uint32_t log_m, uint32_t nd,
                                const uint32_t* dig_bits, int to_natural, hipStream_t s);

hipError_t launch_degree_check(const uint32_t* coef, uint32_t log_m, uint32_t nd, const uint32_t* dig_bits, uint32_t bound, uint32_t* out, hipStream_t s);

hipError_t launch_build_inv_xm1(uint32_t* out, uint32_t logN, PowTable htab, uint32_t shift_mont, hipStream_t s);
hipError_t launch_build_inv_xm1_range(uint32_t* out, size_t count, uint32_t e0, uint32_t log_order, PowTable htab, uint32_t shift_mont, hipStream_t s);
hipError_t launch_halo_pack(const uint32_t* loc, uint32_t* out, uint32_t log_per, uint32_t lg, uint32_t h, hipStream_t s);
hipError_t launch_interleave(const uint32_t* in, uint32_t* out, uint32_t log_parts, uint32_t log_cnt, hipStream_t s);

inline __host__ __device__ uint32_t shard_pattern(uint32_t from, uint32_t to, uint32_t j) {
    uint32_t x = ((from + 1u) * 0x9E3779B1u) ^ ((to + 1u) * 0x85EBCA6Bu) ^ (j * 0xC2B2AE35u + 0x27D4EB2Fu);
    x ^= x >> 15; x *= 0x2C1B3C6Du; x ^= x >> 12;
    return x;
}
hipError_t launch_pattern_fill(uint32_t* dst, uint32_t rank, uint32_t log_per, uint32_t log_parts, hipStream_t s);
hipError_t launch_pattern_check(const uint32_t* src, uint32_t rank, uint32_t log_per, uint32_t log_parts, uint32_t log_chunks, uint32_t* out, hipStream_t s);

struct ComposeArgs {
    const uint32_t* f;
    const uint32_t* inv_xm1;
    uint32_t* cp;
    uint32_t logN, log_b;
    PowTable htab;
    uint32_t w_mont;
    uint32_t gm1_mont, gm2_mont, gm3_mont;
    uint32_t first;
    uint32_t last;
    uint32_t alpha0_mont;
    uint32_t alpha1g2_mont;
    uint32_t zz[32];
};
hipError_t launch_compose(const ComposeArgs& a, hipStream_t s, Profiler* prof = nullptr);

struct ComposeBlockArgs {
    ComposeArgs a;
    const uint32_t* halo;
    uint32_t lg, log_cnt, log_m, halo_stride, e0;
};

struct FoldArgs {
    const uint32_t* in;
    uint32_t* out;
    uint32_t log_m;
    uint32_t round;
    PowTable hinv;
    uint32_t L;
    uint32_t inv2_mont;
    uint32_t c_mont;
    const uint32_t* dyn;
};
hipError_t launch_fri_fold(const FoldArgs& a, hipStream_t s, Profiler* prof = nullptr);

struct FoldMultiArgs {
    const uint32_t* in;
    uint32_t* out;
    uint32_t log_m, round, steps;
    PowTable hinv;
    uint32_t scale_mont;
    uint32_t c_mont[7];
};
hipError_t launch_fri_fold_multi(const FoldMultiArgs& a, hipStream_t s, Profiler* prof = nullptr);
struct FoldMultiBatchArgs {
    FoldMultiArgs a;
    const uint32_t* beta_raw;
    uint32_t beta_stride;
    uint32_t* cb;
    uint32_t batch;
};
hipError_t launch_fri_fold_multi_batch(const FoldMultiBatchArgs& a, hipStream_t s, Profiler* prof = nullptr);

constexpr uint32_t kMailDigests = 16;
struct MailArgs {
    uint32_t* mailbox = nullptr;
    uint32_t seq = 0, top = 0;
    uint32_t* counter = nullptr;
    const uint32_t* dump_src = nullptr;
    uint32_t dump_log = 0;
    uint32_t vals_off = 0;
};
hipError_t launch_merkle_build(const uint32_t* vals, uint32_t log_m, uint32_t* nodes, hipStream_t s, Profiler* prof = nullptr,
                               const MailArgs& mail = MailArgs{}, int hash = 0);
bool set_merkle_latency_log(uint32_t v);
struct ScatterSeg { uint64_t src, dst; uint32_t words, kind; };
hipError_t launch_scatter(const uint32_t* stage, const ScatterSeg* segs, uint32_t count, double words, uint32_t* trees, uint32_t* layers,
                          hipStream_t s, Profiler* prof = nullptr);

hipError_t launch_merkle_build_interleaved(const uint32_t* recv, uint32_t log_parts, uint32_t log_cnt, uint32_t* nodes, hipStream_t s,
                                           Profiler* prof = nullptr, int hash = 0, const MailArgs& mail = MailArgs{});
hipError_t launch_merkle_build_chunk(const uint32_t* recv, uint32_t log_parts, uint32_t log_cnt, uint32_t* nodes, uint32_t log_m,
                                     uint32_t chunk, hipStream_t s, Profiler* prof = nullptr, int hash = 0);
uint32_t merkle_finish_start_depth(uint32_t log_m, uint32_t log_chunks);
hipError_t launch_merkle_finish(uint32_t* nodes, uint32_t log_m, uint32_t log_chunks, hipStream_t s, Profiler* prof = nullptr, int hash = 0,
                                const MailArgs& mail = MailArgs{});
hipError_t launch_fold_merkle(const FoldArgs& a, uint32_t* nodes, hipStream_t s, Profiler* prof = nullptr,
                              const MailArgs& mail = MailArgs{}, int hash = 0);
hipError_t launch_compose_merkle(const ComposeArgs& a, uint32_t* nodes, hipStream_t s, Profiler* prof = nullptr,
                                 const MailArgs& mail = MailArgs{}, int hash = 0);
hipError_t launch_compose_block_merkle(const ComposeBlockArgs& b, uint32_t* nodes, hipStream_t s, Profiler* prof = nullptr,
                                       const MailArgs& mail = MailArgs{}, int hash = 0);

struct BatchChal {
    uint32_t first, last;
    uint32_t alpha0_mont, alpha1g2_mont, alpha2_mont;
    uint32_t c_mont;
    uint32_t pad[2];
};
struct ComposeBatchArgs { ComposeArgs a; const BatchChal* chal; };
struct FoldBatchArgs { FoldArgs a; const BatchChal* chal; };
hipError_t launch_compose_merkle_batch(const ComposeBatchArgs& a, uint32_t log_batch, uint32_t* nodes, hipStream_t s, Profiler* prof,
                                       const MailArgs& mail, int hash);
hipError_t launch_fold_merkle_batch(const FoldBatchArgs& a, uint32_t log_batch, uint32_t* nodes, hipStream_t s, Profiler* prof,
                                    const MailArgs& mail, int hash);
// ... 14 lines not shown
```

zkstark_amd/csrc/ntt_fast.hip:

```cpp
#include "kernels.hpp"

#include "field.hpp"

namespace zk {

namespace {

constexpr uint32_t c_mulmod(uint32_t a, uint32_t b) { return (uint32_t)(((uint64_t)a * b) % P); }
constexpr uint32_t c_powmod(uint32_t a, uint64_t e) {
    uint32_t r = 1, b = a;
    while (e) {
        if (e & 1) r = c_mulmod(r, b);
        b = c_mulmod(b, b);
        e >>= 1;
    }
    return r;
}
constexpr uint32_t c_to_mont(uint32_t a) { return (uint32_t)((((uint64_t)a) << 32) % P); }
constexpr uint32_t kW32 = c_powmod(GEN_W, (uint64_t)(P - 1) >> 5);
constexpr uint32_t kW32Inv = c_powmod(kW32, 31);

template <bool INV>
struct Root32 {
    static constexpr uint32_t w(int e) { return c_to_mont(c_powmod(INV ? kW32Inv : kW32, (uint64_t)e)); }
// ... 176 lines not shown
#pragma unroll
            for (int ta = 0; ta < RA; ++ta) x[ta] = ld_b(srcb, off, in_sgpr((uint32_t)(ta * RB) << row_sh));
        }
        if (MODE != NTT_DIF && logS) {
            uint32_t cur = ONE ? pow_of(pre_cur) : pow_lookup(p.tw, (tb * s) << tw_shift);
            const uint32_t step = ONE ? pow_of(pre_step) : pow_lookup(p.tw, ((uint32_t)RB * s) << tw_shift);
#pragma unroll
            for (int ta = 0; ta < RA; ++ta) {
                x[ta] = mont_mul(x[ta], cur);
                if (ta + 1 < RA) cur = mont_mul(cur, step);
            }
        }
        dft_regs<INV, LA>(x);
#pragma unroll
        for (int i = 0; i < RA; ++i) {
            const int ka = c_brev(i, LA);
            uint32_t v = x[i];
            if (ka != 0) v = mont_mul(v, twl[tb * ka]);
            tile[(ka * RB + tb) * PITCH + c] = v;
        }
    }
    __syncthreads();

#ifndef ZK_NTT_LDE_DIRECT
#define ZK_NTT_LDE_DIRECT 1
#endif
    const bool lde_direct = ZK_NTT_LDE_DIRECT && LDE && logS >= 3;
    constexpr bool TO_LDS = STAGED || LDE;
    uint32_t keep[IT2][RB];
#pragma unroll
    for (int it = 0; it < IT2; ++it) {
        const uint32_t q = tid + it * kThreads;
        if (RA * C < kThreads && q >= (uint32_t)(RA * C)) continue;
        const uint32_t c = q & (C - 1), ka = q >> LOGC;
        uint32_t (&y)[RB] = keep[it];
#pragma unroll
        for (int tb = 0; tb < RB; ++tb) y[tb] = tile[(ka * RB + tb) * PITCH + c];
        dft_regs<INV, LB>(y);
        if (MODE == NTT_DIF) {
            if (logS) {
                uint32_t cur = pow_of(post_cur[it]);
                const uint32_t step = pow_of(post_step[it]);
#pragma unroll
                for (int kb = 0; kb < RB; ++kb) {
                    const int i = c_brev(kb, LB);
                    y[i] = mont_mul(y[i], cur);
                    if (kb + 1 < RB) cur = mont_mul(cur, step);
                }
            } else if (p.scale_mont) {
#pragma unroll
                for (int i = 0; i < RB; ++i) y[i] = mont_mul(y[i], p.scale_mont);
            }
        }
        if (!TO_LDS) {
            const uint32_t off = (ka << row_sh) + (c << 2);
#pragma unroll
            for (int i = 0; i < RB; ++i) st_b(dstb, off, in_sgpr((uint32_t)(RA * c_brev(i, LB)) << row_sh), y[i]);
        } else if (ZK_NTT_LDE_DIRECT && LDE && lde_direct) {
            const uint32_t off = ((c >> logS) << (LOGR + logS + 2)) + (ka << row_sh) + ((c & smask) << 2);
#pragma unroll
            for (int i = 0; i < RB; ++i) st_b(tdst, off, in_sgpr((uint32_t)(RA * c_brev(i, LB)) << row_sh), y[i]);
        }
    }
    if (TO_LDS && !lde_direct) {
        __syncthreads();
#pragma unroll
        for (int it = 0; it < IT2; ++it) {
            const uint32_t q = tid + it * kThreads;
            if (RA * C < kThreads && q >= (uint32_t)(RA * C)) continue;
            const uint32_t c = q & (C - 1), ka = q >> LOGC;
#pragma unroll
            for (int i = 0; i < RB; ++i) tile[(ka + RA * c_brev(i, LB)) * PITCH + c] = keep[it][i];
        }
        __syncthreads();
#pragma unroll 4
        for (uint32_t l = tid; l < (uint32_t)(R * C); l += kThreads) {
            uint32_t s = l & smask, t = (l >> logS) & (R - 1), c = ((l >> (LOGR + logS)) << logS) | s;
            st_b(tdst, l << 2, 0, tile[t * PITCH + c]);
        }
    }
}

template <uint32_t MODE, int LA, int LB, int TILE_LOG>
hipError_t launch3(const NttPassArgs& a, bool staged, uint32_t blocks, hipStream_t s) {
    constexpr int R = 1 << (LA + LB), C = 1 << (TILE_LOG - LA - LB);
    size_t shmem = ((size_t)R * (C + 1) + R) * sizeof(uint32_t);
    const dim3 grid(blocks, a.batch ? a.batch : 1);
    if (MODE == NTT_DIT_LDE && a.prep) {
        if (a.logS >= 1) {
            shmem += (size_t)(C >> a.logS) * (R + 1) * sizeof(uint32_t);
            hipLaunchKernelGGL((ntt_pass_fast_kernel<MODE, LA, LB, true, TILE_LOG, MODE == NTT_DIT_LDE ? 2 : 0>), grid, dim3(kThreads), shmem, s, a);
        } else {
            hipLaunchKernelGGL((ntt_pass_fast_kernel<MODE, LA, LB, true, TILE_LOG, MODE == NTT_DIT_LDE ? 1 : 0>), grid, dim3(kThreads), shmem, s, a);
        }
    }
    else if (staged) hipLaunchKernelGGL((ntt_pass_fast_kernel<MODE, LA, LB, true, TILE_LOG, 0>), grid, dim3(kThreads), shmem, s, a);
    else hipLaunchKernelGGL((ntt_pass_fast_kernel<MODE, LA, LB, false, TILE_LOG, 0>), grid, dim3(kThreads), shmem, s, a);
    return hipGetLastError();
}

template <uint32_t MODE, int LA, int LB>
hipError_t launch2(const NttPassArgs& a, bool staged, uint32_t blocks, hipStream_t s) {
    return a.tile_log == kSmallTileLog ? launch3<MODE, LA, LB, (int)kSmallTileLog>(a, staged, blocks, s)
                                       : launch3<MODE, LA, LB, (int)kMidTileLog>(a, staged, blocks, s);
}

template <uint32_t MODE>
hipError_t launch1(const NttPassArgs& a, bool staged, uint32_t blocks, hipStream_t s) {
    switch (a.logR) {
        case 5: return launch2<MODE, 3, 2>(a, staged, blocks, s);
        case 6: return launch2<MODE, 3, 3>(a, staged, blocks, s);
        case 7: return launch2<MODE, 4, 3>(a, staged, blocks, s);
        case 8: return launch2<MODE, 4, 4>(a, staged, blocks, s);
    }
    return hipErrorInvalidValue;
}

}

bool ntt_fast_ok(const NttPassArgs& a, NttMode mode) {
    if (a.logR < 5 || a.logR > 8) return false;
    if (a.tile_log != kSmallTileLog && a.tile_log != kMidTileLog) return false;
    const uint32_t logC = a.tile_log - a.logR;
    if (a.log_total < a.tile_log || a.logC != logC) return false;
    if (mode == NTT_DIT_LDE && !(a.logS < logC)) return false;
    return true;
}

bool launch_ntt_pass_fast(const NttPassArgs& a, NttMode mode, hipStream_t s, hipError_t* err) {
    if (!ntt_fast_ok(a, mode)) return false;
    const bool staged = a.logS < a.tile_log - a.logR;
    const uint32_t blocks = 1u << (a.log_total - a.tile_log);
    switch (mode) {
        case NTT_DIF: *err = launch1<NTT_DIF>(a, staged, blocks, s); break;
        case NTT_DIT: *err = launch1<NTT_DIT>(a, staged, blocks, s); break;
        case NTT_DIT_LDE: *err = launch1<NTT_DIT_LDE>(a, true, blocks, s); break;
    }
    return true;
}

}
```

zkstark_amd/csrc/zkstark.hip:

```cpp
#include <hip/hip_runtime.h>

#include <algorithm>
#include <chrono>
#include <cstdarg>
#include <cstdio>
#include <cstdlib>
#include <cstring>
#include <atomic>
#include <condition_variable>
#include <functional>
#include <mutex>
#include <new>
#include <thread>
#include <string>
#include <vector>

#include "../../include/zkstark_amd.h"
#include "field.hpp"
#include "kernels.hpp"
#include "sha256.hpp"
#include "transcript.hpp"
#include "host_sha.hpp"
#include "internal.hpp"
#include "pool.hpp"

using namespace zk;
using namespace zk::impl;

struct zk_ctx {
    int device = 0;
    uint32_t log_n = 0, log_b = 0, L = 0;
    size_t n = 0, N = 0, B = 0;
    uint32_t R = 0;
    hipStream_t stream = nullptr;
    zk_dom* dom = nullptr;
    uint32_t* d_trace = nullptr;
    uint32_t* d_coef = nullptr;
    uint32_t* d_layers = nullptr;
    std::vector<size_t> layer_off, layer_len;
    uint32_t* d_trees = nullptr;
    std::vector<size_t> tree_off;
    uint64_t* d_gather_off = nullptr;
    uint32_t* d_gather_out = nullptr;
    uint64_t* h_gather_off = nullptr;
    uint32_t* h_gather_out = nullptr;
    uint64_t* dm_gather_off = nullptr;
    uint32_t* dm_gather_out = nullptr;
    const uint32_t* host_nodes[40] = {};
    size_t host_node_cnt[40] = {};
    const uint32_t* host_vals[40] = {};
    std::vector<const uint32_t*> fetch_vals, fetch_nodes;
    std::vector<uint32_t> fetch_vdev;
    std::vector<uint64_t> fetch_ditems;
    std::vector<uint8_t> commit_buf;
    bool pending_top = false;
    uint32_t pending_tree = 0;
    size_t open_nv = 0, open_ndg = 0, open_vi = 0;
    bool open_pending = false;
    uint32_t* h_small = nullptr;
    uint32_t* h_mailbox = nullptr;
    uint32_t* d_mailbox = nullptr;
    uint32_t* d_counter = nullptr;
    bool counters_dirty = false;
    uint32_t mail_seq = 0;
    uint32_t tree_seq[40] = {};
    bool early = false, early_ok = false, gate_pending = false;
    uint32_t* h_gate = nullptr;
    uint32_t* d_gate = nullptr;
    uint32_t* h_dyn = nullptr;
    uint32_t* d_dyn = nullptr;
    uint32_t gate_seq = 0;
    uint32_t host_top = 0, host_tail = 0;
    Pool* pool = nullptr;
    uint32_t* h_stage = nullptr;
    uint32_t* d_stage = nullptr;
    size_t stage_words = 0, stage_used = 0;
    ScatterSeg* h_segs = nullptr;
    ScatterSeg* d_segs = nullptr;
    uint32_t n_segs = 0;
    double seg_words = 0;
    std::vector<uint32_t> tail_vals;
    uint32_t tail_log = 0;
    bool tail_have = false;
    double t_wait = 0, t_host_hash = 0, t_launch = 0;
    bool tail = false;
    uint32_t hinv_host = 0;
    uint32_t queries = 1;
    uint32_t grind = 0;
    Grinder* grinder = nullptr;
    uint32_t fold = 1;
    uint64_t skipped_layers = 0, skipped_trees = 0;
    int hash = 0;
    bool checks = false;
    uint32_t* d_check = nullptr;
    DevTable ones;
    size_t gather_cap = 0;
    size_t device_bytes = 0;
    double setup_ms = 0;
    bool have_trace = false, have_lde = false;
    uint32_t first = 0, last = 0;
    zk_transcript_info info{};
    Profiler prof;
    zk_kernel_stat kstat[K_COUNT] = {};
};

namespace {

template <typename T>
int dmalloc(zk_ctx* c, T** p, size_t bytes) {
    hipError_t e = hipMalloc((void**)p, bytes ? bytes : 4);
    if (e != hipSuccess) return fail(ZK_ERR_NOMEM, "hipMalloc(%zu) failed: %s", bytes, hipGetErrorString(e));
    c->device_bytes += bytes;
    return ZK_OK;
}

size_t layer_size(const zk_ctx* c, uint32_t layer) { return layer == 0 ? c->N : (c->N >> (layer - 1)); }
uint32_t layer_log(const zk_ctx* c, uint32_t layer) { return layer == 0 ? c->L : c->L - (layer - 1); }

Profiler* prof_of(zk_ctx* c) { return c->prof.mask ? &c->prof : nullptr; }

void collect_kernel_stats(zk_ctx* c) {
    for (auto& r : c->prof.recs) {
        float ms = 0;
        (void)hipEventSynchronize(r.b);
        (void)hipEventElapsedTime(&ms, r.a, r.b);
        c->kstat[r.cls].launches += 1;
        c->kstat[r.cls].ms += ms;
        c->kstat[r.cls].bytes += r.bytes;
        c->kstat[r.cls].ops += r.ops;
        c->prof.pool.push_back(r.a);
        c->prof.pool.push_back(r.b);
    }
    c->prof.recs.clear();
}

int do_lde(zk_ctx* c) {
    int rc = dom_lde(c->dom, c->d_trace, c->d_coef, c->d_layers + c->layer_off[0], c->stream, prof_of(c));
    if (!rc) c->have_lde = true;
    return rc;
}

#ifndef ZK_HOST_SUB_LOG
#define ZK_HOST_SUB_LOG 8
#endif
static_assert(ZK_HOST_SUB_LOG >= 4 && ZK_HOST_SUB_LOG <= (int)kMaxHostLog, "host sub-tree size");
constexpr uint32_t host_sub_log() { return ZK_HOST_SUB_LOG; }
uint32_t top_of(const zk_ctx* c, uint32_t tree) {
    if (c->hash != 0 || !c->host_top) return 0;
    const uint32_t lg = layer_log(c, tree);
    return lg > c->host_top ? c->host_top : lg - 1;
}
MailArgs mail_of(zk_ctx* c, uint32_t tree, bool host, bool feed_tail = true) {
    MailArgs m;
    if (c->counters_dirty) {
        (void)hipMemsetAsync(c->d_counter, 0, 64, c->stream);
        c->counters_dirty = false;
    }
    m.mailbox = c->d_mailbox;
    m.seq = ++c->mail_seq;
    c->tree_seq[tree] = m.seq;
    m.counter = c->d_counter;
    m.top = host ? top_of(c, tree) : 0;
    if (feed_tail && c->fold == 1 && m.top && c->host_tail && tree >= 1 && layer_log(c, tree) == c->host_tail + 1) {
        m.dump_src = c->d_layers + c->layer_off[tree];
        m.dump_log = c->host_tail + 1;
        m.vals_off = (uint32_t)kMailValsOff;
        c->tail_log = m.dump_log;
        c->tail_have = true;
    }
    return m;
}

int do_merkle(zk_ctx* c, uint32_t layer, bool host = false, bool feed_tail = true) {
    HIPCHK(launch_merkle_build(c->d_layers + c->layer_off[layer], layer_log(c, layer), c->d_trees + c->tree_off[layer], c->stream,
                               prof_of(c), mail_of(c, layer, host, feed_tail), c->hash));
    return ZK_OK;
}

int do_compose_commit(zk_ctx* c, const uint32_t alpha_raw[3]) {
    ComposeArgs a;
    int rc = compose_args(c->dom, c->d_layers + c->layer_off[0], c->d_layers + c->layer_off[1], c->first, c->last, alpha_raw, a);
    if (rc) return rc;
    HIPCHK(launch_compose_merkle(a, c->d_trees + c->tree_off[1], c->stream, prof_of(c), mail_of(c, 1, true), c->hash));
    return ZK_OK;
}
int do_fold_commit(zk_ctx* c, uint32_t round, uint32_t beta_raw) {
    FoldArgs a;
    int rc = fold_args(c->dom, c->d_layers + c->layer_off[1 + round], c->d_layers + c->layer_off[2 + round], c->L - round, round, beta_raw, a);
    if (rc) return rc;
    HIPCHK(launch_fold_merkle(a, c->d_trees + c->tree_off[2 + round], c->stream, prof_of(c), mail_of(c, 2 + round, true), c->hash));
// ... 231 lines not shown
void open_path(zk_ctx* c, uint32_t tree, size_t m, size_t leaf) {
    for (size_t i = leaf + m - 1; i != 0; i = (i - 1) >> 1) {
        const size_t nd = (i & 1) ? i + 1 : i - 1;
        if (nd < c->host_node_cnt[tree]) c->fetch_nodes.push_back(c->host_nodes[tree] + 8 * nd);
        else { c->fetch_nodes.push_back(c->h_gather_out + 8 * c->open_ndg); ++c->open_ndg; c->fetch_ditems.push_back((uint64_t)c->tree_off[tree] + (uint64_t)nd * 8); }
    }
}
int open_launch(zk_ctx* c) {
    const size_t nv = c->open_nv, ndg = c->open_ndg;
    if (nv + ndg > c->gather_cap) return fail(ZK_ERR_STATE, "gather capacity exceeded");
    if (ndg) memcpy(c->h_gather_off + nv, c->fetch_ditems.data(), ndg * 8);
    for (size_t i = 0; i < c->fetch_vals.size(); ++i)
        if (!c->fetch_vals[i]) c->fetch_vals[i] = c->h_gather_out + 8 * ndg + c->fetch_vdev[i];
    c->open_pending = nv + ndg != 0;
    if (c->open_pending)
        HIPCHK(launch_fetch(c->d_layers, c->d_trees, c->dm_gather_off, (uint32_t)nv, (uint32_t)ndg, c->dm_gather_out, c->d_mailbox,
                            ++c->mail_seq, c->d_counter, c->stream, prof_of(c)));
    return ZK_OK;
}
int open_wait(zk_ctx* c) {
    if (!c->open_pending) return ZK_OK;
    c->open_pending = false;
    return wait_mail(c, c->mail_seq);
}

int prove_fold_rounds(zk_ctx* c, Channel& ch) {
    const uint32_t R = c->R, K = c->fold;
    uint8_t root[32];
    int rc;
    for (uint32_t r0 = 0; r0 < R; r0 += K) {
        const uint32_t steps = R - r0 < K ? R - r0 : K, id = 1 + r0 + steps;
        const uint32_t beta = c->info.beta_raw[r0] = ch.get_u32();
        if ((rc = dom_fold_multi(c->dom, c->d_layers + c->layer_off[1 + r0], c->d_layers + c->layer_off[id], c->L - r0, r0, steps, beta,
                                 c->stream, prof_of(c)))) return rc;
        if ((rc = do_merkle(c, id, true, false))) return rc;
        if ((rc = read_commit(c, id, root))) return rc;
        const size_t deg = c->n >> (r0 + steps);
        if (c->checks && (rc = check_degree(c, id, (uint32_t)deg - (deg ? 1 : 0), "prover.rs:228-251 (FRI layer degree)"))) return rc;
        ch.commit_hash(root);
        memcpy(c->info.roots[id], root, 32);
        for (uint32_t l = 2 + r0; l < id; ++l) { c->skipped_layers |= (uint64_t)1 << l; c->skipped_trees |= (uint64_t)1 << l; }
    }
    return ZK_OK;
}

struct HostLaps {
    const bool on;
    std::chrono::steady_clock::time_point t0 = std::chrono::steady_clock::now();
    void operator()(const char* what) {
        if (!on) return;
        auto t = std::chrono::steady_clock::now();
        fprintf(stderr, "[zk timing] %-28s %8.1f us\n", what, std::chrono::duration<double, std::micro>(t - t0).count());
        t0 = t;
    }
};

int prove_finish(zk_ctx* c, Channel& ch, HostLaps& lap) {
    const uint32_t R = c->R, K = c->fold, Q = c->queries, G = fold_groups(R, K);
    const size_t B = c->B, N = c->N, Lp = c->L;
    int rc;
    uint32_t free_term = 0;
    if ((rc = last_layer_value(c, &free_term))) return rc;
    c->info.free_term = free_term;
    ch.commit_u32(free_term);
    if (c->grind) {
        uint64_t w = 0;
        if ((rc = grind_channel(c->grinder, ch, c->grind, &w))) return rc;
        c->info.grind_bits = c->grind;
        c->info.grind_nonce = w;
        lap("grind");
    }
    uint32_t qraws[64];
    for (uint32_t k = 0; k < Q; ++k) qraws[k] = ch.get_u32();
    c->info.query_raw = qraws[0];

    size_t per_query = 0;
    for_each_opening(c->log_n, c->log_b, K, 0, [&](uint32_t, uint32_t, size_t) { ++per_query; });
    open_begin(c, (size_t)Q * per_query);
    for (uint32_t k = 0; k < Q; ++k)
        for_each_opening(c->log_n, c->log_b, K, (size_t)qraws[k] % (N - 2 * B), [&](uint32_t layer, uint32_t log_len, size_t leaf) {
            open_val(c, layer, leaf); open_path(c, layer, (size_t)1 << log_len, leaf);
        });
    if ((rc = open_launch(c))) return rc;
    if ((rc = flush_host_parts(c))) return rc;
    lap("free term + fetch enqueue");
    if ((rc = open_wait(c))) return rc;
    lap("fetch wait");
    const uint32_t* const* vsrc = c->fetch_vals.data();
    const uint32_t* const* dsrc = c->fetch_nodes.data();
    std::vector<uint8_t>& buf = c->commit_buf;
    buf.resize(Channel::group_bytes((size_t)1 << fold_steps(R, K, 0), Lp));
    auto tuple = [&](size_t s, size_t plen) {
        ch.commit_group(buf.data(), s, plen, [&](size_t t) { return *vsrc[t]; },
                        [&](size_t i, uint8_t* out) { digest_words_to_bytes(dsrc[i], out); });
        vsrc += s; dsrc += s * plen;
    };
    for (uint32_t q = 0; q < Q; ++q) {
        for (int k = 0; k < 4; ++k) tuple(1, Lp);
        for (uint32_t j = 0; j < G; ++j) tuple((size_t)1 << fold_steps(R, K, j), Lp - (size_t)j * K);
    }
    lap("decommit host hashing");
    return ZK_OK;
}

int prove_resident(zk_ctx* c, Channel& ch) {
    if (!c->have_trace) return fail(ZK_ERR_STATE, "zk_prove_resident: no trace uploaded");
    static const bool timing = getenv("ZK_HOST_TIMING") != nullptr;
    HostLaps lap{timing};
    const uint32_t R = c->R;
    ch.data.reserve(ch.data.size() + proof_data_len(c->log_n, c->log_b, c->queries, c->grind, c->fold));
    c->skipped_layers = c->skipped_trees = 0;
    uint8_t root[32];
    int rc;
    memset(&c->info, 0, sizeof c->info);
    c->info.public_last = c->last;
    c->pending_top = false;
    begin_proof(c);
    GateGuard gate_guard{c};
    if ((rc = do_lde(c))) return rc;
    if (c->checks && ((rc = checks_alloc(c)) || (rc = check_interpolant(c)))) return rc;
    if ((rc = do_merkle(c, 0, true))) return rc;
    if ((rc = read_commit(c, 0, root))) return rc;
    ch.commit_hash(root);
    memcpy(c->info.roots[0], root, 32);
    uint32_t alpha[3];
    for (int i = 0; i < 3; ++i) alpha[i] = c->info.alpha_raw[i] = ch.get_u32();
    if ((rc = do_compose_commit(c, alpha))) return rc;
    if (can_gate(c, 0) && (rc = enqueue_gated_fold(c, 0))) return rc;
    if ((rc = read_commit(c, 1, root))) return rc;
    if (c->checks && (rc = check_degree(c, 1, (uint32_t)c->n - 1, "prover.rs:148-159/:169 (exact divisions, deg cp = n - 1)"))) return rc;
    ch.commit_hash(root);
    memcpy(c->info.roots[1], root, 32);
    if (c->fold > 1) {
        if ((rc = prove_fold_rounds(c, ch))) return rc;
    } else for (uint32_t r = 0; r < R; ++r) {
        uint32_t beta = c->info.beta_raw[r] = ch.get_u32();
        if (c->gate_pending) {
            release_gated_fold(c, r, beta);
            if (can_gate(c, r + 1) && (rc = enqueue_gated_fold(c, r + 1))) return rc;
            if ((rc = read_commit(c, 2 + r, root))) return rc;
        } else if (c->tail_have && c->tail_log == c->L - r && c->L - r - 1 <= c->host_tail) {
            if ((rc = host_fold_commit(c, r, beta, root))) return rc;
        } else {
            if ((rc = do_fold_commit(c, r, beta))) return rc;
            if (can_gate(c, r + 1) && (rc = enqueue_gated_fold(c, r + 1))) return rc;
            if ((rc = read_commit(c, 2 + r, root))) return rc;
        }
        if (c->checks && (rc = check_degree(c, 2 + r, (uint32_t)(c->n >> (r + 1)) - ((c->n >> (r + 1)) ? 1 : 0), "prover.rs:228-251 (FRI layer degree)"))) return rc;
        ch.commit_hash(root);
        memcpy(c->info.roots[2 + r], root, 32);
    }
    lap("lde .. last root");
    if (timing) fprintf(stderr, "[zk timing]   of which: waiting for the device %.1f us, host hashing (tops + tail) %.1f us\n", c->t_wait, c->t_host_hash);
    return prove_finish(c, ch, lap);
}

}

namespace zk {
namespace impl {
int tail_open_begin(zk_ctx* c, size_t x) {
    if (!c || !c->tail) return fail(ZK_ERR_INVALID, "tail_open_begin: not a tail context");
    HIPCHK(hipSetDevice(c->device));
    open_begin(c, 2 * (size_t)c->R);
    for (uint32_t i = 0; i < c->R; ++i) {
        const size_t len = c->N >> i, xi = x % len, nx = (xi + len / 2) % len;
        open_val(c, 1 + i, xi); open_path(c, 1 + i, len, xi);
// ... 295 lines not shown

int zk_ctx_set_host_levels(zk_ctx* c, uint32_t top_log, uint32_t tail_log) {
    if (!c) return fail(ZK_ERR_INVALID, "null context");
    if (top_log > kMaxHostLog || tail_log > kMaxHostLog || (tail_log && !top_log))
        return fail(ZK_ERR_INVALID, "zk_ctx_set_host_levels: need top_log, tail_log <= %u, and top_log > 0 when tail_log > 0", kMaxHostLog);
    c->host_top = top_log;
    c->host_tail = tail_log;
    return ctx_team(c);
}
int zk_ctx_get_host_levels(const zk_ctx* c, uint32_t* top_log, uint32_t* tail_log) {
    if (!c || !top_log || !tail_log) return fail(ZK_ERR_INVALID, "zk_ctx_get_host_levels: null argument");
    *top_log = c->host_top;
    *tail_log = c->host_tail;
    return ZK_OK;
}
int zk_ctx_set_checks(zk_ctx* c, int on) {
    if (!c) return fail(ZK_ERR_INVALID, "null context");
    if (c->tail) return fail(ZK_ERR_STATE, "zk_ctx_set_checks: FRI-tail context");
    c->checks = on != 0;
    return ZK_OK;
}
int zk_ctx_set_hash(zk_ctx* c, int hash_kind) {
    if (!c) return fail(ZK_ERR_INVALID, "null context");
    if (hash_kind != ZK_HASH_SHA256 && hash_kind != ZK_HASH_FIELD) return fail(ZK_ERR_INVALID, "zk_ctx_set_hash: unknown hash %d", hash_kind);
    c->hash = hash_kind;
    return ZK_OK;
}

int zk_ctx_set_profiling(zk_ctx* c, uint32_t class_mask) {
    if (!c) return fail(ZK_ERR_INVALID, "null context");
    c->prof.mask = class_mask & ((1u << K_COUNT) - 1u);
    return ZK_OK;
}

static int put_kernel_stats(zk_kernel_stat* out, size_t count, const zk_kernel_stat* src, const char* who) {
    if (!count) return ZK_OK;
    const uint32_t stride = out[0].struct_size;
    if (!abi_bytes(out, who)) return ZK_ERR_INVALID;
    for (size_t i = 0; i < count && i < (size_t)K_COUNT; ++i) {
        zk_kernel_stat* o = reinterpret_cast<zk_kernel_stat*>(reinterpret_cast<char*>(out) + i * stride);
        o->struct_size = stride;
        if (int rc = abi_put(o, src[i], who)) return rc;
    }
    return ZK_OK;
}

int zk_kernel_stats(zk_ctx* c, zk_kernel_stat* out, size_t count, int reset) {
    if (!c || (!out && count)) return fail(ZK_ERR_INVALID, "zk_kernel_stats: null argument");
    collect_kernel_stats(c);
    if (int rc = put_kernel_stats(out, count, c->kstat, "zk_kernel_stats")) return rc;
    if (reset) for (int i = 0; i < K_COUNT; ++i) c->kstat[i] = zk_kernel_stat{};
    return ZK_OK;
}

int zk_trace_fibsq(uint32_t a0, uint32_t a1, size_t count, uint32_t* out) {
    if (!out && count) return fail(ZK_ERR_INVALID, "zk_trace_fibsq: out is null");
    if (count > 0) out[0] = a0 % P;
    if (count > 1) out[1] = a1 % P;
    for (size_t i = 2; i < count; ++i)
        out[i] = add(mulmod(out[i - 2], out[i - 2]), mulmod(out[i - 1], out[i - 1]));
    return ZK_OK;
}

int zk_trace_upload(zk_ctx* c, const uint32_t* trace, size_t count) {
    if (!c || !trace) return fail(ZK_ERR_INVALID, "zk_trace_upload: null argument");
    if (count != c->n - 1) return fail(ZK_ERR_INVALID, "zk_trace_upload: expected n-1 = %zu values, got %zu", c->n - 1, count);
    for (size_t i = 0; i < count; ++i)
        if (trace[i] >= P) return fail(ZK_ERR_INVALID, "zk_trace_upload: trace[%zu] = %u is not a canonical residue", i, trace[i]);
    HIPCHK(hipSetDevice(c->device));
    HIPCHK(hipMemcpyAsync(c->d_trace, trace, count * 4, hipMemcpyHostToDevice, c->stream));
    HIPCHK(hipMemsetAsync(c->d_trace + count, 0, 4, c->stream));
    HIPCHK(hipStreamSynchronize(c->stream));
    c->first = trace[0];
    c->last = trace[count - 1];
    c->have_trace = true;
    c->have_lde = false;
    return ZK_OK;
}

int zk_lde(zk_ctx* c) {
    if (!c) return fail(ZK_ERR_INVALID, "null context");
    if (!c->have_trace) return fail(ZK_ERR_STATE, "zk_lde: no trace uploaded");
    HIPCHK(hipSetDevice(c->device));
    static const bool timing = getenv("ZK_HOST_TIMING") != nullptr;
    const double t0 = now_us();
    int rc = do_lde(c);
    if (timing) fprintf(stderr, "[zk timing] lde: enqueue of %u passes %.1f us\n", 2 * c->dom->plan.nd, now_us() - t0);
    return rc;
}

int zk_merkle_commit(zk_ctx* c, uint32_t layer, uint8_t root_out[32]) {
    if (!c || !root_out) return fail(ZK_ERR_INVALID, "zk_merkle_commit: null argument");
    if (layer > c->R + 1) return fail(ZK_ERR_INVALID, "zk_merkle_commit: layer %u out of range", layer);
    HIPCHK(hipSetDevice(c->device));
    static const bool timing = getenv("ZK_HOST_TIMING") != nullptr;
    const double t0 = now_us();
    c->skipped_trees &= ~((uint64_t)1 << layer);
    if (c->pending_top && c->pending_tree == layer) c->pending_top = false;
    int rc = settle_pending(c);
    if (rc) return rc;
    begin_proof(c);
    rc = do_merkle(c, layer, true, false);
    const double t1 = now_us();
    if (!rc) rc = read_commit(c, layer, root_out);
    const double t2 = now_us();
    if (!rc && c->n_segs) { c->pending_top = true; c->pending_tree = layer; }
    if (timing)
        fprintf(stderr, "[zk timing] merkle_commit(layer %u): enqueue %.1f us, wait for the device %.1f us, host top %.1f us, scatter enqueue %.1f us\n",
                layer, t1 - t0, c->t_wait, c->t_host_hash, now_us() - t2);
    return rc;
}

int zk_compose(zk_ctx* c, const uint32_t alpha_raw[3]) {
    if (!c || !alpha_raw) return fail(ZK_ERR_INVALID, "zk_compose: null argument");
    if (!c->have_lde) return fail(ZK_ERR_STATE, "zk_compose: run zk_lde first");
    HIPCHK(hipSetDevice(c->device));
    return do_compose(c, alpha_raw);
}

int zk_fri_fold(zk_ctx* c, uint32_t round, uint32_t beta_raw) {
    if (!c) return fail(ZK_ERR_INVALID, "null context");
    if (round >= c->R) return fail(ZK_ERR_INVALID, "zk_fri_fold: round %u out of range (%u rounds)", round, c->R);
    HIPCHK(hipSetDevice(c->device));
    c->skipped_layers &= ~((uint64_t)1 << (2 + round));
    return do_fold(c, round, beta_raw);
}
int zk_fri_fold_multi(zk_ctx* c, uint32_t round, uint32_t steps, uint32_t beta_raw) {
    if (!c) return fail(ZK_ERR_INVALID, "null context");
    if (steps < 1 || steps > kMaxFoldLog) return fail(ZK_ERR_INVALID, "zk_fri_fold_multi: steps must be 1..%u (got %u)", kMaxFoldLog, steps);
    if (round >= c->R || round + steps > c->R) return fail(ZK_ERR_INVALID, "zk_fri_fold_multi: rounds %u..%u out of range (%u rounds)", round, round + steps, c->R);
    HIPCHK(hipSetDevice(c->device));
    c->skipped_layers &= ~((uint64_t)1 << (1 + round + steps));
    return dom_fold_multi(c->dom, c->d_layers + c->layer_off[1 + round], c->d_layers + c->layer_off[1 + round + steps], c->L - round, round, steps,
                          beta_raw, c->stream, prof_of(c));
}

int zk_layer_read(zk_ctx* c, uint32_t layer, size_t offset, size_t count, uint32_t* out) {
    if (!c || (!out && count)) return fail(ZK_ERR_INVALID, "zk_layer_read: null argument");
    if (layer > c->R + 1 || offset + count > layer_size(c, layer)) return fail(ZK_ERR_INVALID, "zk_layer_read: out of range");
    if ((c->skipped_layers >> layer) & 1) return fail(ZK_ERR_STATE, "zk_layer_read: layer %u was not materialised by the last proof (fold_log %u)", layer, c->fold);
    HIPCHK(hipSetDevice(c->device));
    if (int prc = settle_pending(c)) return prc;
    HIPCHK(hipMemcpyAsync(out, c->d_layers + c->layer_off[layer] + offset, count * 4, hipMemcpyDeviceToHost, c->stream));
    HIPCHK(hipStreamSynchronize(c->stream));
    return ZK_OK;
}

int zk_layer_write(zk_ctx* c, uint32_t layer, size_t offset, size_t count, const uint32_t* in) {
    if (!c || (!in && count)) return fail(ZK_ERR_INVALID, "zk_layer_write: null argument");
    if (layer > c->R + 1 || offset + count > layer_size(c, layer)) return fail(ZK_ERR_INVALID, "zk_layer_write: out of range");
    for (size_t i = 0; i < count; ++i)
        if (in[i] >= P) return fail(ZK_ERR_INVALID, "zk_layer_write: value %zu is not a canonical residue", i);
    HIPCHK(hipSetDevice(c->device));
    HIPCHK(hipMemcpyAsync(c->d_layers + c->layer_off[layer] + offset, in, count * 4, hipMemcpyHostToDevice, c->stream));
    HIPCHK(hipStreamSynchronize(c->stream));
    if (layer == 0) c->have_lde = true;
    c->skipped_layers &= ~((uint64_t)1 << layer);
    return ZK_OK;
}

int zk_merkle_node(zk_ctx* c, uint32_t tree, size_t index, uint8_t out[32]) {
    if (!c || !out) return fail(ZK_ERR_INVALID, "zk_merkle_node: null argument");
    if (tree > c->R + 1 || index >= 2 * layer_size(c, tree) - 1) return fail(ZK_ERR_INVALID, "zk_merkle_node: out of range");
    if ((c->skipped_trees >> tree) & 1) return fail(ZK_ERR_STATE, "zk_merkle_node: tree %u was not built by the last proof (fold_log %u)", tree, c->fold);
    HIPCHK(hipSetDevice(c->device));
    if (int prc = settle_pending(c)) return prc;
    HIPCHK(hipMemcpyAsync(c->h_small, c->d_trees + c->tree_off[tree] + index * 8, 32, hipMemcpyDeviceToHost, c->stream));
    HIPCHK(hipStreamSynchronize(c->stream));
    digest_words_to_bytes(c->h_small, out);
    return ZK_OK;
}

int zk_merkle_nodes(zk_ctx* c, uint32_t tree, size_t first, size_t count, uint8_t* out) {
    if (!c || (!out && count)) return fail(ZK_ERR_INVALID, "zk_merkle_nodes: null argument");
    if (tree > c->R + 1 || first > 2 * layer_size(c, tree) - 1 || count > 2 * layer_size(c, tree) - 1 - first)
        return fail(ZK_ERR_INVALID, "zk_merkle_nodes: out of range");
    if ((c->skipped_trees >> tree) & 1) return fail(ZK_ERR_STATE, "zk_merkle_nodes: tree %u was not built by the last proof (fold_log %u)", tree, c->fold);
    HIPCHK(hipSetDevice(c->device));
    if (int prc = settle_pending(c)) return prc;
    return merkle_nodes_to_host(c->device, c->stream, c->d_trees + c->tree_off[tree], first, count, out);
}

int zk_merkle_path(zk_ctx* c, uint32_t tree, size_t leaf, uint8_t* out, size_t* path_len) {
    if (!c || !out) return fail(ZK_ERR_INVALID, "zk_merkle_path: null argument");
    if (tree > c->R + 1 || leaf >= layer_size(c, tree)) return fail(ZK_ERR_INVALID, "zk_merkle_path: out of range");
    if ((c->skipped_trees >> tree) & 1) return fail(ZK_ERR_STATE, "zk_merkle_path: tree %u was not built by the last proof (fold_log %u)", tree, c->fold);
    HIPCHK(hipSetDevice(c->device));
    if (int prc = settle_pending(c)) return prc;
    std::vector<size_t> nodes;
    path_nodes(layer_size(c, tree), leaf, nodes);
    for (size_t i = 0; i < nodes.size(); ++i) c->h_gather_off[i] = (uint64_t)c->tree_off[tree] + (uint64_t)nodes[i] * 8;
    HIPCHK(hipMemcpyAsync(c->d_gather_off, c->h_gather_off, nodes.size() * 8, hipMemcpyHostToDevice, c->stream));
    HIPCHK(launch_gather(c->d_trees, c->d_gather_off, (uint32_t)nodes.size(), 8, c->d_gather_out, c->stream));
    HIPCHK(hipMemcpyAsync(c->h_gather_out, c->d_gather_out, nodes.size() * 32, hipMemcpyDeviceToHost, c->stream));
    HIPCHK(hipStreamSynchronize(c->stream));
    for (size_t i = 0; i < nodes.size(); ++i) digest_words_to_bytes(c->h_gather_out + 8 * i, out + 32 * i);
    if (path_len) *path_len = nodes.size();
    return ZK_OK;
}

int zk_prove_resident(zk_ctx* c, uint8_t* proof_out, size_t cap, size_t* proof_len, uint8_t state_out[32]) {
    if (!c || !proof_out || !state_out) return fail(ZK_ERR_INVALID, "zk_prove_resident: null argument");
    HIPCHK(hipSetDevice(c->device));
    Channel ch;
    int rc = prove_resident(c, ch);
    if (rc) return rc;
    const std::vector<uint8_t>& proof = ch.data;
    if (proof_len) *proof_len = proof.size();
    if (proof.size() > cap) return fail(ZK_ERR_BUFFER, "zk_prove: proof needs %zu bytes, buffer has %zu", proof.size(), cap);
    memcpy(proof_out, proof.data(), proof.size());
    memcpy(state_out, ch.state, 32);
    return ZK_OK;
}

int zk_prove_channel(zk_ctx* c, zk_channel* chan) {
    if (!c || !chan) return fail(ZK_ERR_INVALID, "zk_prove_channel: null argument");
    if (c->tail) return fail(ZK_ERR_STATE, "zk_prove_channel: FRI-tail context");
    HIPCHK(hipSetDevice(c->device));
    return prove_resident(c, chan->ch);
}

int zk_prove(zk_ctx* c, const uint32_t* trace, size_t count, uint8_t* proof_out, size_t cap, size_t* proof_len,
             uint8_t state_out[32]) {
    int rc = zk_trace_upload(c, trace, count);
    if (rc) return rc;
    return zk_prove_resident(c, proof_out, cap, proof_len, state_out);
}

int zk_prove_many(zk_ctx* const* ctxs, size_t count, uint8_t* proofs_out, size_t stride, size_t* lens_out, uint8_t* states_out) {
    if (!ctxs || !proofs_out || !lens_out || !states_out || count == 0 || count > 16)
        return fail(ZK_ERR_INVALID, "zk_prove_many: need 1..16 contexts and non-null outputs");
    for (size_t i = 0; i < count; ++i) {
        if (!ctxs[i]) return fail(ZK_ERR_INVALID, "zk_prove_many: context %zu is null", i);
        for (size_t j = 0; j < i; ++j)
            if (ctxs[j] == ctxs[i]) return fail(ZK_ERR_INVALID, "zk_prove_many: context %zu appears twice", i);
    }
// ... 639 lines not shown
```

Baseline: 2.933 billion.

## Precompute vanishing-ratio table, simplify fold math, defer host flush, batch timer launches

Adds a per-domain precomputed table vz holding the cubic boundary polynomial times the inverse of the x^n-1 denominator, so the compose kernel loads one extra word per element instead of evaluating the polynomial and looking up powers. FRI fold replaces the multiply by inverse-2 with a shift-based halving and folds the challenge constant into the x-inverse factor, using a wave-uniform fast path. The proof's final host-part flush is deferred into a pending state that later API calls settle. Kernel launches are also routed through the scoped timer object. The cost is one extra N-sized device buffer, extra memory traffic in compose, and more complex pending-state handling.

```diff
diff --git a/zkstark_amd/csrc/domain.hip b/zkstark_amd/csrc/domain.hip
--- a/zkstark_amd/csrc/domain.hip
+++ b/zkstark_amd/csrc/domain.hip
@@ -92,6 +92,7 @@
     if (!d) return;
     free_table(&d->H); free_table(&d->Hinv); free_table(&d->W);
     if (d->d_inv_xm1) (void)hipFree(d->d_inv_xm1);
+    if (d->d_vz) (void)hipFree(d->d_vz);
     delete d;
 }
 
@@ -136,6 +137,17 @@
         e = launch_build_inv_xm1(d->d_inv_xm1, d->L, d->H.view(), d->shift_mont, stream);
         if (e == hipSuccess) e = hipStreamSynchronize(stream);
         if (e != hipSuccess) { dom_free(d); return fail(ZK_ERR_HIP, "inv_xm1 build failed: %s", hipGetErrorString(e)); }
+        bool den_ok = true;
+        uint32_t zden[32] = {0};
+        for (size_t r = 0; r < d->B; ++r) { den_ok = den_ok && d->inv_den[r] != 0; zden[r] = to_mont(to_mont(d->inv_den[r])); }
+        if (den_ok) {
+            e = hipMalloc((void**)&d->d_vz, d->N * 4);
+            if (e != hipSuccess) { dom_free(d); return fail(ZK_ERR_NOMEM, "hipMalloc(%zu) failed", d->N * 4); }
+            d->device_bytes += d->N * 4;
+            e = launch_build_vz(d->d_vz, d->L, d->log_b, d->H.view(), d->shift_mont, d->gm1_mont, d->gm2_mont, d->gm3_mont, zden, stream);
+            if (e == hipSuccess) e = hipStreamSynchronize(stream);
+            if (e != hipSuccess) { dom_free(d); return fail(ZK_ERR_HIP, "vz build failed: %s", hipGetErrorString(e)); }
+        }
     }
     *out = d;
     return ZK_OK;
@@ -184,7 +196,7 @@
 int compose_args(const zk_dom* d, const uint32_t* d_f, uint32_t* d_cp, uint32_t first, uint32_t last,
                  const uint32_t alpha_raw[3], ComposeArgs& a) {
     a = ComposeArgs{};
-    a.f = d_f; a.inv_xm1 = d->d_inv_xm1; a.cp = d_cp;
+    a.f = d_f; a.inv_xm1 = d->d_inv_xm1; a.vz = d->d_vz; a.cp = d_cp;
     a.logN = d->L; a.log_b = d->log_b;
     a.htab = d->H.view();
     a.w_mont = d->shift_mont; a.gm1_mont = d->gm1_mont; a.gm2_mont = d->gm2_mont; a.gm3_mont = d->gm3_mont;
@@ -192,6 +204,7 @@
     uint32_t a0 = alpha_raw[0] % P, a1 = alpha_raw[1] % P, a2 = alpha_raw[2] % P;
     a.alpha0_mont = to_mont(a0);
     a.alpha1g2_mont = to_mont(mulmod(a1, mulmod(d->g, d->g)));
+    a.alpha2_mont = to_mont(a2);
     for (size_t r = 0; r < d->B; ++r) {
         if (d->inv_den[r] == 0) return fail(ZK_ERR_INVALID, "compose: x^n = 1 on the domain");
         a.zz[r] = to_mont(to_mont(mulmod(a2, d->inv_den[r])));
diff --git a/zkstark_amd/csrc/internal.hpp b/zkstark_amd/csrc/internal.hpp
--- a/zkstark_amd/csrc/internal.hpp
+++ b/zkstark_amd/csrc/internal.hpp
@@ -115,6 +115,7 @@
     uint32_t shift = 0, g = 0, h = 0;
     zk::impl::DevTable H, Hinv, W;
     uint32_t* d_inv_xm1 = nullptr;
+    uint32_t* d_vz = nullptr;
     zk::impl::Plan plan;
     uint32_t shift_mont = 0, gm1_mont = 0, gm2_mont = 0, gm3_mont = 0, ninv_mont = 0, inv2_mont = 0;
     uint32_t fold_k[32] = {0};
diff --git a/zkstark_amd/csrc/kernels.hip b/zkstark_amd/csrc/kernels.hip
--- a/zkstark_amd/csrc/kernels.hip
+++ b/zkstark_amd/csrc/kernels.hip
@@ -135,7 +135,7 @@
     }
 }
 
-bool launch_ntt_pass_fast(const NttPassArgs& a, NttMode mode, hipStream_t s, hipError_t* err);
+bool launch_ntt_pass_fast(const NttPassArgs& a, NttMode mode, ScopedKernelTimer& tm, hipError_t* err);
 
 hipError_t launch_ntt_pass(const NttPassArgs& a, NttMode mode, hipStream_t s, Profiler* prof) {
     double bytes = mode == NTT_DIT_LDE ? 4.0 * ((double)((size_t)1 << (a.log_total - a.logS)) + (double)((size_t)1 << a.log_total))
@@ -143,14 +143,14 @@
     const uint32_t batch = a.batch ? a.batch : 1;
     ScopedKernelTimer tm(prof, K_NTT, bytes * batch, s, kNttOpsPerElement * (double)((size_t)1 << a.log_total) * batch * (double)a.logR / 7.0);
     hipError_t ferr = hipSuccess;
-    if (launch_ntt_pass_fast(a, mode, s, &ferr)) return ferr;
+    if (launch_ntt_pass_fast(a, mode, tm, &ferr)) return ferr;
     uint32_t cols_log = a.log_total - a.logR;
     uint32_t blocks = 1u << (cols_log - a.logC);
     size_t shmem = ((size_t)(1u << a.logR) * ((1u << a.logC) + 1u) + (1u << a.logR) / 2u) * sizeof(uint32_t);
     switch (mode) {
-        case NTT_DIF: hipLaunchKernelGGL(ntt_pass_kernel<NTT_DIF>, dim3(blocks, batch), dim3(kNttThreads), shmem, s, a); break;
-        case NTT_DIT: hipLaunchKernelGGL(ntt_pass_kernel<NTT_DIT>, dim3(blocks, batch), dim3(kNttThreads), shmem, s, a); break;
-        case NTT_DIT_LDE: hipLaunchKernelGGL(ntt_pass_kernel<NTT_DIT_LDE>, dim3(blocks, batch), dim3(kNttThreads), shmem, s, a); break;
+        case NTT_DIF: tm.launch(ntt_pass_kernel<NTT_DIF>, dim3(blocks, batch), dim3(kNttThreads), shmem, a); break;
+        case NTT_DIT: tm.launch(ntt_pass_kernel<NTT_DIT>, dim3(blocks, batch), dim3(kNttThreads), shmem, a); break;
+        case NTT_DIT_LDE: tm.launch(ntt_pass_kernel<NTT_DIT_LDE>, dim3(blocks, batch), dim3(kNttThreads), shmem, a); break;
     }
     return hipGetLastError();
 }
@@ -175,7 +175,7 @@
                                uint32_t batch, size_t u_stride, size_t out_stride) {
     uint32_t n = 1u << a.log_n;
     ScopedKernelTimer tm(prof, K_NTT, 8.0 * n * batch, s);
-    hipLaunchKernelGGL(coef_prepare_kernel, dim3((n + 255) / 256, batch), dim3(256), 0, s, U, out, a, u_stride, out_stride);
+    tm.launch(coef_prepare_kernel, dim3((n + 255) / 256, batch), dim3(256), 0, U, out, a, u_stride, out_stride);
     return hipGetLastError();
 }
 
@@ -268,7 +268,26 @@
     return launch_build_inv_xm1_range(out, (size_t)1 << logN, 0u, logN, htab, shift_mont, s);
 }
 
-struct ComposeRaw { uint32_t f0, f1, f2, inv0, inv2, x_hi, x_lo, zz; };
+struct VzArgs { uint32_t* out; uint32_t logN, log_b; PowTable htab; uint32_t w_mont, gm1_mont, gm2_mont, gm3_mont; uint32_t zden[32]; };
+__global__ __launch_bounds__(256) void build_vz_kernel(VzArgs a) {
+    const size_t i = (size_t)blockIdx.x * blockDim.x + threadIdx.x;
+    if (i >= ((size_t)1 << a.logN)) return;
+    const uint32_t x = mont_mul(pow_lookup(a.htab, (uint32_t)i), a.w_mont);
+    const uint32_t v3 = mont_mul(mont_mul(sub(x, a.gm3_mont), sub(x, a.gm2_mont)), sub(x, a.gm1_mont));
+    a.out[i] = mont_mul(v3, a.zden[i & ((1u << a.log_b) - 1u)]);
+}
+hipError_t launch_build_vz(uint32_t* out, uint32_t logN, uint32_t log_b, PowTable htab, uint32_t shift_mont, uint32_t gm1_mont, uint32_t gm2_mont,
+                           uint32_t gm3_mont, const uint32_t* zden, hipStream_t s) {
+    VzArgs a{};
+    a.out = out; a.logN = logN; a.log_b = log_b; a.htab = htab;
+    a.w_mont = shift_mont; a.gm1_mont = gm1_mont; a.gm2_mont = gm2_mont; a.gm3_mont = gm3_mont;
+    for (uint32_t r = 0; r < (1u << log_b); ++r) a.zden[r] = zden[r];
+    const size_t N = (size_t)1 << logN;
+    hipLaunchKernelGGL(build_vz_kernel, dim3((uint32_t)((N + 255) / 256)), dim3(256), 0, s, a);
+    return hipGetLastError();
+}
+
+struct ComposeRaw { uint32_t f0, f1, f2, inv0, inv2, vz; };
 __device__ __forceinline__ ComposeRaw compose_fetch(const ComposeArgs& a, const uint32_t* f, size_t i) {
     const size_t N = (size_t)1 << a.logN;
     const uint32_t B = 1u << a.log_b;
@@ -276,35 +295,35 @@
     ComposeRaw r;
     r.f0 = f[i]; r.f1 = f[i1]; r.f2 = f[i2];
     r.inv0 = a.inv_xm1[i]; r.inv2 = a.inv_xm1[i2];
-    r.x_hi = a.htab.hi[(uint32_t)i >> a.htab.lo_bits]; r.x_lo = a.htab.lo[(uint32_t)i & ((1u << a.htab.lo_bits) - 1u)];
-    r.zz = a.zz[i & (B - 1)];
+    r.vz = a.vz[i];
     return r;
 }
-template <bool BATCH>
-__device__ __forceinline__ uint32_t compose_eval(const ComposeArgs& a, uint32_t f0, uint32_t f1, uint32_t f2, uint32_t inv0, uint32_t inv2,
-                                                 uint32_t x, uint32_t zz, uint32_t first, uint32_t last, uint32_t al0, uint32_t al1g2, uint32_t al2) {
+__device__ __forceinline__ uint32_t compose_sum(uint32_t f0, uint32_t f1, uint32_t f2, uint32_t inv0, uint32_t inv2, uint32_t y,
+                                                uint32_t first, uint32_t last, uint32_t al0, uint32_t al1g2) {
     uint32_t t0 = mont_mul(mont_mul(sub(f0, first), inv0), al0);
     uint32_t t1 = mont_mul(mont_mul(sub(f0, last), inv2), al1g2);
-    uint32_t v3 = mont_mul(mont_mul(sub(x, a.gm3_mont), sub(x, a.gm2_mont)), sub(x, a.gm1_mont));
-    uint32_t y = mont_mul(v3, zz);
-    if (BATCH) y = mont_mul(y, al2);
     uint32_t num = sub(sub(mont_mul(f2, 1u), mont_mul(f1, f1)), mont_mul(f0, f0));
     uint32_t t2 = mont_mul(num, y);
     return add(add(t0, t1), t2);
 }
-template <bool BATCH>
-__device__ __forceinline__ uint32_t compose_finish(const ComposeArgs& a, const ComposeRaw& r, uint32_t first, uint32_t last, uint32_t al0,
-                                                   uint32_t al1g2, uint32_t al2) {
-    const uint32_t x = mont_mul(mont_mul(r.x_hi, r.x_lo), a.w_mont);
-    return compose_eval<BATCH>(a, r.f0, r.f1, r.f2, r.inv0, r.inv2, x, r.zz, first, last, al0, al1g2, al2);
-}
-template <bool BATCH>
+__device__ __forceinline__ uint32_t compose_eval(uint32_t f0, uint32_t f1, uint32_t f2, uint32_t inv0, uint32_t inv2, uint32_t vz,
+                                                 uint32_t first, uint32_t last, uint32_t al0, uint32_t al1g2, uint32_t al2) {
+    return compose_sum(f0, f1, f2, inv0, inv2, mont_mul(vz, al2), first, last, al0, al1g2);
+}
+__device__ __forceinline__ uint32_t compose_eval_x(const ComposeArgs& a, uint32_t f0, uint32_t f1, uint32_t f2, uint32_t inv0, uint32_t inv2,
+                                                   uint32_t x, uint32_t zz) {
+    uint32_t v3 = mont_mul(mont_mul(sub(x, a.gm3_mont), sub(x, a.gm2_mont)), sub(x, a.gm1_mont));
+    return compose_sum(f0, f1, f2, inv0, inv2, mont_mul(v3, zz), a.first, a.last, a.alpha0_mont, a.alpha1g2_mont);
+}
+__device__ __forceinline__ uint32_t compose_finish(const ComposeRaw& r, uint32_t first, uint32_t last, uint32_t al0, uint32_t al1g2, uint32_t al2) {
+    return compose_eval(r.f0, r.f1, r.f2, r.inv0, r.inv2, r.vz, first, last, al0, al1g2, al2);
+}
 __device__ __forceinline__ uint32_t compose_core(const ComposeArgs& a, const uint32_t* f, uint32_t first, uint32_t last, uint32_t al0,
                                                  uint32_t al1g2, uint32_t al2, size_t i) {
-    return compose_finish<BATCH>(a, compose_fetch(a, f, i), first, last, al0, al1g2, al2);
+    return compose_finish(compose_fetch(a, f, i), first, last, al0, al1g2, al2);
 }
 __device__ __forceinline__ uint32_t compose_at(const ComposeArgs& a, size_t i) {
-    return compose_core<false>(a, a.f, a.first, a.last, a.alpha0_mont, a.alpha1g2_mont, 0u, i);
+    return compose_core(a, a.f, a.first, a.last, a.alpha0_mont, a.alpha1g2_mont, a.alpha2_mont, i);
 }
 
 __global__ __launch_bounds__(256) void compose_kernel(ComposeArgs a) {
@@ -320,8 +339,9 @@
     if (i >= N) return;
     const uint4* fv = reinterpret_cast<const uint4*>(a.f);
     const uint4* iv = reinterpret_cast<const uint4*>(a.inv_xm1);
-    uint32_t f0[4], f1[4], f2[4], inv0[4], inv2[4], zz[4];
-    const uint4 v0 = fv[i >> 2], w0 = iv[i >> 2];
+    uint32_t f0[4], f1[4], f2[4], inv0[4], inv2[4];
+    const uint4 v0 = fv[i >> 2], w0 = iv[i >> 2], z0 = reinterpret_cast<const uint4*>(a.vz)[i >> 2];
+    const uint32_t vz[4] = {z0.x, z0.y, z0.z, z0.w};
     f0[0] = v0.x; f0[1] = v0.y; f0[2] = v0.z; f0[3] = v0.w;
     inv0[0] = w0.x; inv0[1] = w0.y; inv0[2] = w0.z; inv0[3] = w0.w;
     if (B >= 4) {
@@ -329,9 +349,6 @@
         f1[0] = v1.x; f1[1] = v1.y; f1[2] = v1.z; f1[3] = v1.w;
         f2[0] = v2.x; f2[1] = v2.y; f2[2] = v2.z; f2[3] = v2.w;
         inv2[0] = w2.x; inv2[1] = w2.y; inv2[2] = w2.z; inv2[3] = w2.w;
-        const uint32_t z0 = (uint32_t)i & (B - 1);
-#pragma unroll
-        for (int k = 0; k < 4; ++k) zz[k] = a.zz[z0 + k];
     } else {
         const uint4 v1 = fv[((i + 4) & (N - 1)) >> 2], w1 = iv[((i + 4) & (N - 1)) >> 2];
         const uint32_t fw[8] = {v0.x, v0.y, v0.z, v0.w, v1.x, v1.y, v1.z, v1.w};
@@ -341,30 +358,26 @@
             f1[k] = B == 1 ? fw[k + 1] : fw[k + 2];
             f2[k] = B == 1 ? fw[k + 2] : fw[k + 4];
             inv2[k] = B == 1 ? iw[k + 2] : iw[k + 4];
-            zz[k] = B == 1 ? a.zz[0] : a.zz[k & 1];
-        }
-    }
-    uint32_t x = mont_mul(pow_lookup(a.htab, (uint32_t)i), a.w_mont);
-    const uint32_t h = pow_lookup(a.htab, 1u);
+        }
+    }
     uint32_t r[4];
 #pragma unroll
-    for (int k = 0; k < 4; ++k) {
-        r[k] = compose_eval<false>(a, f0[k], f1[k], f2[k], inv0[k], inv2[k], x, zz[k], a.first, a.last, a.alpha0_mont, a.alpha1g2_mont, 0u);
-        if (k < 3) x = mont_mul(x, h);
-    }
+    for (int k = 0; k < 4; ++k)
+        r[k] = compose_eval(f0[k], f1[k], f2[k], inv0[k], inv2[k], vz[k], a.first, a.last, a.alpha0_mont, a.alpha1g2_mont, a.alpha2_mont);
     reinterpret_cast<uint4*>(a.cp)[i >> 2] = make_uint4(r[0], r[1], r[2], r[3]);
 }
 
 hipError_t launch_compose(const ComposeArgs& a, hipStream_t s, Profiler* prof) {
     size_t N = (size_t)1 << a.logN;
     ScopedKernelTimer tm(prof, K_COMPOSE, 8.0 * (double)N, s);
-    const bool aligned = ((reinterpret_cast<uintptr_t>(a.f) | reinterpret_cast<uintptr_t>(a.inv_xm1) | reinterpret_cast<uintptr_t>(a.cp)) & 15u) == 0;
+    const bool aligned = ((reinterpret_cast<uintptr_t>(a.f) | reinterpret_cast<uintptr_t>(a.inv_xm1) | reinterpret_cast<uintptr_t>(a.vz) |
+                           reinterpret_cast<uintptr_t>(a.cp)) & 15u) == 0;
     if (a.logN >= 4 && aligned) {
         uint32_t blocks = (uint32_t)((N / 4 + 255) / 256);
-        hipLaunchKernelGGL(compose_kernel4, dim3(blocks), dim3(256), 0, s, a);
+        tm.launch(compose_kernel4, dim3(blocks), dim3(256), 0, a);
     } else {
         uint32_t blocks = (uint32_t)((N + 255) / 256);
-        hipLaunchKernelGGL(compose_kernel, dim3(blocks), dim3(256), 0, s, a);
+        tm.launch(compose_kernel, dim3(blocks), dim3(256), 0, a);
     }
     return hipGetLastError();
 }
@@ -378,10 +391,14 @@
     r.x_hi = a.hinv.hi[e >> a.hinv.lo_bits]; r.x_lo = a.hinv.lo[e & ((1u << a.hinv.lo_bits) - 1u)];
     return r;
 }
+__device__ __forceinline__ uint32_t halve(uint32_t t) { return (t >> 1) + ((t & 1u) ? (P >> 1) + 1u : 0u); }
 __device__ __forceinline__ uint32_t fold_finish(const FoldArgs& a, const FoldRaw& r) {
-    uint32_t xinv = mont_mul(r.x_hi, r.x_lo);
-    uint32_t s = mont_mul(add(r.u, r.v), a.inv2_mont);
-    uint32_t d = mont_mul(mont_mul(sub(r.u, r.v), xinv), a.c_mont);
+    const uint32_t hi0 = __builtin_amdgcn_readfirstlane(r.x_hi);
+    uint32_t k;
+    if (__builtin_amdgcn_ballot_w64(r.x_hi != hi0) == 0) k = mont_mul(hi0, a.c_mont);
+    else k = mont_mul(r.x_hi, a.c_mont);
+    uint32_t s = halve(add(r.u, r.v));
+    uint32_t d = mont_mul(mont_mul(sub(r.u, r.v), k), r.x_lo);
     return add(s, d);
 }
 __device__ __forceinline__ uint32_t fold_at(const FoldArgs& a, size_t i) { return fold_finish(a, fold_fetch(a, i)); }
@@ -398,15 +415,13 @@
     if (i >= half) return;
     const uint4 u = reinterpret_cast<const uint4*>(a.in)[i >> 2], v = reinterpret_cast<const uint4*>(a.in)[(i + half) >> 2];
     const uint32_t uu[4] = {u.x, u.y, u.z, u.w}, vv[4] = {v.x, v.y, v.z, v.w};
-    uint32_t xinv = pow_lookup(a.hinv, (uint32_t)(i << a.round));
+    uint32_t xc = mont_mul(pow_lookup(a.hinv, (uint32_t)(i << a.round)), a.c_mont);
     const uint32_t step = pow_lookup(a.hinv, 1u << a.round);
     uint32_t r[4];
 #pragma unroll
     for (int k = 0; k < 4; ++k) {
-        const uint32_t sm = mont_mul(add(uu[k], vv[k]), a.inv2_mont);
-        const uint32_t d = mont_mul(mont_mul(sub(uu[k], vv[k]), xinv), a.c_mont);
-        r[k] = add(sm, d);
-        if (k < 3) xinv = mont_mul(xinv, step);
+        r[k] = add(halve(add(uu[k], vv[k])), mont_mul(sub(uu[k], vv[k]), xc));
+        if (k < 3) xc = mont_mul(xc, step);
     }
     reinterpret_cast<uint4*>(a.out)[i >> 2] = make_uint4(r[0], r[1], r[2], r[3]);
 }
@@ -417,10 +432,10 @@
     const bool aligned = ((reinterpret_cast<uintptr_t>(a.in) | reinterpret_cast<uintptr_t>(a.out)) & 15u) == 0;
     if (half >= 4 && aligned) {
         uint32_t blocks = (uint32_t)((half / 4 + 255) / 256);
-        hipLaunchKernelGGL(fri_fold_kernel4, dim3(blocks), dim3(256), 0, s, a);
+        tm.launch(fri_fold_kernel4, dim3(blocks), dim3(256), 0, a);
     } else {
         uint32_t blocks = (uint32_t)((half + 255) / 256);
-        hipLaunchKernelGGL(fri_fold_kernel, dim3(blocks), dim3(256), 0, s, a);
+        tm.launch(fri_fold_kernel, dim3(blocks), dim3(256), 0, a);
     }
     return hipGetLastError();
 }
@@ -481,18 +496,18 @@
 }
 
 template <int STEPS>
-static void fold_multi_launch(const FoldMultiArgs& a, size_t q, bool wide, hipStream_t s) {
-    if (wide) hipLaunchKernelGGL(fri_fold_multi_kernel<STEPS>, dim3((uint32_t)((q / 4 + 255) / 256)), dim3(256), 0, s, a);
-    else hipLaunchKernelGGL(fri_fold_multi_kernel1<STEPS>, dim3((uint32_t)((q + 255) / 256)), dim3(256), 0, s, a);
+static void fold_multi_launch(ScopedKernelTimer& tm, const FoldMultiArgs& a, size_t q, bool wide) {
+    if (wide) tm.launch(fri_fold_multi_kernel<STEPS>, dim3((uint32_t)((q / 4 + 255) / 256)), dim3(256), 0, a);
+    else tm.launch(fri_fold_multi_kernel1<STEPS>, dim3((uint32_t)((q + 255) / 256)), dim3(256), 0, a);
 }
 hipError_t launch_fri_fold_multi(const FoldMultiArgs& a, hipStream_t s, Profiler* prof) {
     if (a.steps < 1 || a.steps > 3 || a.log_m < a.steps) return hipErrorInvalidValue;
     const size_t m = (size_t)1 << a.log_m, q = m >> a.steps;
     ScopedKernelTimer tm(prof, K_FOLD, 4.0 * (double)(m + q), s);
     const bool wide = q >= 4 && ((reinterpret_cast<uintptr_t>(a.in) | reinterpret_cast<uintptr_t>(a.out)) & 15u) == 0;
-    if (a.steps == 1) fold_multi_launch<1>(a, q, wide, s);
-    else if (a.steps == 2) fold_multi_launch<2>(a, q, wide, s);
-    else fold_multi_launch<3>(a, q, wide, s);
+    if (a.steps == 1) fold_multi_launch<1>(tm, a, q, wide);
+    else if (a.steps == 2) fold_multi_launch<2>(tm, a, q, wide);
+    else fold_multi_launch<3>(tm, a, q, wide);
     return hipGetLastError();
 }
 
@@ -577,7 +592,7 @@
     if (a.steps < 1 || a.steps > 3 || a.log_m < a.steps || a.log_m > 32 || p.batch < 1 || !p.beta_raw || !p.cb) return hipErrorInvalidValue;
     const size_t m = (size_t)1 << a.log_m, q = m >> a.steps, total = (size_t)p.batch * q;
     if ((size_t)p.batch * m > ((size_t)1 << 32)) return hipErrorInvalidValue;
-    ScopedKernelTimer tm(prof, K_FOLD, 4.0 * (double)p.batch * (double)(m + q), s);
+    ScopedKernelTimer tm(prof, K_FOLD, 4.0 * (double)p.batch * (double)(m + q), s, 0.0, true);
     const bool wide = q >= 4 && ((reinterpret_cast<uintptr_t>(a.in) | reinterpret_cast<uintptr_t>(a.out)) & 15u) == 0;
     if (a.steps == 1) fold_multi_batch_launch<1>(p, total, wide, s);
     else if (a.steps == 2) fold_multi_batch_launch<2>(p, total, wide, s);
@@ -614,11 +629,22 @@
     __device__ __forceinline__ uint32_t finish(const Raw& r, size_t pos) const { uint32_t v = fold_finish(a, r); a.out[pos] = v; return v; }
     __device__ __forceinline__ uint32_t load(size_t pos) const { return finish(fetch(pos), pos); }
 };
+#ifndef ZK_COMPOSE_FETCH_AHEAD
+#define ZK_COMPOSE_FETCH_AHEAD 0
+#endif
 struct ComposeSrc {
     ComposeArgs a;
+#if ZK_COMPOSE_FETCH_AHEAD
+    using Raw = ComposeRaw;
+    __device__ __forceinline__ Raw fetch(size_t pos) const { return compose_fetch(a, a.f, pos); }
+    __device__ __forceinline__ uint32_t finish(const Raw& r, size_t pos) const {
+        uint32_t v = compose_finish(r, a.first, a.last, a.alpha0_mont, a.alpha1g2_mont, a.alpha2_mont); a.cp[pos] = v; return v;
+    }
+#else
     using Raw = size_t;
     __device__ __forceinline__ Raw fetch(size_t pos) const { return pos; }
     __device__ __forceinline__ uint32_t finish(const Raw& r, size_t) const { return load(r); }
+#endif
     __device__ __forceinline__ uint32_t load(size_t pos) const { uint32_t v = compose_at(a, pos); a.cp[pos] = v; return v; }
 };
 
@@ -642,8 +668,7 @@
         const size_t B = (size_t)1 << a.log_b;
         const uint32_t f0 = f_at(pos), f1 = f_at(pos + B), f2 = f_at(pos + 2 * B);
         const uint32_t x = mont_mul(pow_lookup(a.htab, b.e0 + (uint32_t)pos), a.w_mont);
-        return compose_eval<false>(a, f0, f1, f2, a.inv_xm1[pos], a.inv_xm1[pos + 2 * B], x, a.zz[pos & (B - 1)], a.first, a.last, a.alpha0_mont,
-                                   a.alpha1g2_mont, 0u);
+        return compose_eval_x(a, f0, f1, f2, a.inv_xm1[pos], a.inv_xm1[pos + 2 * B], x, a.zz[pos & (B - 1)]);
     }
 };
 
@@ -656,7 +681,7 @@
     __device__ __forceinline__ uint32_t load(size_t pos) const {
         const size_t b = pos >> a.logN, i = pos & (((size_t)1 << a.logN) - 1);
         const BatchChal c = chal[b];
-        uint32_t v = compose_core<true>(a, a.f + (b << a.logN), c.first, c.last, c.alpha0_mont, c.alpha1g2_mont, c.alpha2_mont, i);
+        uint32_t v = compose_core(a, a.f + (b << a.logN), c.first, c.last, c.alpha0_mont, c.alpha1g2_mont, c.alpha2_mont, i);
         a.cp[pos] = v;
         return v;
     }
@@ -673,7 +698,7 @@
         const uint32_t* in = a.in + (b << a.log_m);
         uint32_t u = in[i], v = in[i + half];
         uint32_t xinv = pow_lookup(a.hinv, (uint32_t)(i << a.round));
-        uint32_t s = mont_mul(add(u, v), a.inv2_mont);
+        uint32_t s = halve(add(u, v));
         uint32_t d = mont_mul(mont_mul(sub(u, v), xinv), chal[b].c_mont);
         uint32_t r = add(s, d);
         a.out[pos] = r;
@@ -1227,11 +1252,11 @@
         size_t sh = (size_t)(kMerkleThreads / 64) * (k + 1) * 128 * sizeof(uint4);
         ScopedKernelTimer tm(prof, leaf ? K_MERKLE_LEAF : K_MERKLE_INNER, first_bytes(merkle_bytes(leaf, depth - stop, k)), s, merkle_ops(leaf, depth - stop, k, hash));
         if (hash) {
-            if (leaf) hipLaunchKernelGGL((merkle_subtree_kernel<SRC, true, 1>), dim3(blocks), dim3(kMerkleThreads), sh, s, src, nodes, depth, k, off_at(depth));
-            else hipLaunchKernelGGL((merkle_subtree_kernel<PlainSrc, false, 1>), dim3(blocks), dim3(kMerkleThreads), sh, s, none, nodes, depth, k, off_at(depth));
+            if (leaf) tm.launch((merkle_subtree_kernel<SRC, true, 1>), dim3(blocks), dim3(kMerkleThreads), sh, src, nodes, depth, k, off_at(depth));
+            else tm.launch((merkle_subtree_kernel<PlainSrc, false, 1>), dim3(blocks), dim3(kMerkleThreads), sh, none, nodes, depth, k, off_at(depth));
         } else {
-            if (leaf) hipLaunchKernelGGL((merkle_subtree_kernel<SRC, true, 0>), dim3(blocks), dim3(kMerkleThreads), sh, s, src, nodes, depth, k, off_at(depth));
-            else hipLaunchKernelGGL((merkle_subtree_kernel<PlainSrc, false, 0>), dim3(blocks), dim3(kMerkleThreads), sh, s, none, nodes, depth, k, off_at(depth));
+            if (leaf) tm.launch((merkle_subtree_kernel<SRC, true, 0>), dim3(blocks), dim3(kMerkleThreads), sh, src, nodes, depth, k, off_at(depth));
+            else tm.launch((merkle_subtree_kernel<PlainSrc, false, 0>), dim3(blocks), dim3(kMerkleThreads), sh, none, nodes, depth, k, off_at(depth));
         }
         leaf = false;
         depth -= k;
@@ -1248,11 +1273,11 @@
         ScopedKernelTimer tm(prof, K_MERKLE_TOP, first_bytes(merkle_bytes(leaf, span, j)) + (j2 ? merkle_bytes(false, span - j, j2) : 0.0), s,
                              merkle_ops(leaf, span, j, hash) + (j2 ? merkle_ops(false, span - j, j2, hash) : 0.0));
         if (hash) {
-            if (leaf) hipLaunchKernelGGL((merkle_wg_kernel<SRC, true, 1>), dim3(blocks), dim3(kWgThreads), sh, s, src, nodes, depth, j, mail, off_at(depth), j2, lds_log);
-            else hipLaunchKernelGGL((merkle_wg_kernel<PlainSrc, false, 1>), dim3(blocks), dim3(kWgThreads), sh, s, none, nodes, depth, j, mail, off_at(depth), j2, lds_log);
+            if (leaf) tm.launch((merkle_wg_kernel<SRC, true, 1>), dim3(blocks), dim3(kWgThreads), sh, src, nodes, depth, j, mail, off_at(depth), j2, lds_log);
+            else tm.launch((merkle_wg_kernel<PlainSrc, false, 1>), dim3(blocks), dim3(kWgThreads), sh, none, nodes, depth, j, mail, off_at(depth), j2, lds_log);
         } else {
-            if (leaf) hipLaunchKernelGGL((merkle_wg_kernel<SRC, true, 0>), dim3(blocks), dim3(kWgThreads), sh, s, src, nodes, depth, j, mail, off_at(depth), j2, lds_log);
-            else hipLaunchKernelGGL((merkle_wg_kernel<PlainSrc, false, 0>), dim3(blocks), dim3(kWgThreads), sh, s, none, nodes, depth, j, mail, off_at(depth), j2, lds_log);
+            if (leaf) tm.launch((merkle_wg_kernel<SRC, true, 0>), dim3(blocks), dim3(kWgThreads), sh, src, nodes, depth, j, mail, off_at(depth), j2, lds_log);
+            else tm.launch((merkle_wg_kernel<PlainSrc, false, 0>), dim3(blocks), dim3(kWgThreads), sh, none, nodes, depth, j, mail, off_at(depth), j2, lds_log);
         }
         leaf = false;
         depth -= j + j2;
@@ -1350,7 +1375,7 @@
                           hipStream_t s, Profiler* prof) {
     if (!count) return hipSuccess;
     ScopedKernelTimer tm(prof, K_GATHER, 8.0 * words, s);
-    hipLaunchKernelGGL(scatter_kernel, dim3(count), dim3(1024), 0, s, stage, segs, trees, layers);
+    tm.launch(scatter_kernel, dim3(count), dim3(1024), 0, stage, segs, trees, layers);
     return hipGetLastError();
 }
 
@@ -1578,7 +1603,7 @@
     if (!count) return hipSuccess;
     ScopedKernelTimer tm(prof, K_GATHER, 8.0 * (double)count * words, s);
     uint32_t total = count * words, blocks = (total + 255) / 256;
-    hipLaunchKernelGGL(gather_kernel, dim3(blocks), dim3(256), 0, s, src, offsets, count, words, out);
+    tm.launch(gather_kernel, dim3(blocks), dim3(256), 0, src, offsets, count, words, out);
     return hipGetLastError();
 }
 
@@ -1615,8 +1640,8 @@
     uint32_t blocks = (work + kFetchThreads - 1) / kFetchThreads;
     if (blocks == 0) blocks = 1;
     if (blocks > 64) blocks = 64;
-    hipLaunchKernelGGL(fetch_kernel, dim3(blocks), dim3(kFetchThreads), 0, s, layers, trees, items, nv, ndg, out, mailbox, seq, counter);
-    return hipGetLastError();
-}
-
-}
+    tm.launch(fetch_kernel, dim3(blocks), dim3(kFetchThreads), 0, layers, trees, items, nv, ndg, out, mailbox, seq, counter);
+    return hipGetLastError();
+}
+
+}
diff --git a/zkstark_amd/csrc/kernels.hpp b/zkstark_amd/csrc/kernels.hpp
--- a/zkstark_amd/csrc/kernels.hpp
+++ b/zkstark_amd/csrc/kernels.hpp
@@ -1,8 +1,10 @@
 #pragma once
 #include <hip/hip_runtime.h>
+#include <hip/hip_ext.h>
 #include <stddef.h>
 #include <stdint.h>
 
+#include <type_traits>
 #include <vector>
 
 namespace zk {
@@ -24,6 +26,13 @@
 constexpr double kFieldLeafOps = 5015.0;
 constexpr double kFieldInnerOps = 5072.0;
 
+enum BracketMode : int { BR_EVENTS = 0, BR_NOFENCE = 1, BR_DISPATCH = 2 };
+#ifndef ZK_PROFILE_BRACKETS
+#define ZK_PROFILE_BRACKETS 0
+#endif
+constexpr BracketMode kBracketMode = (BracketMode)ZK_PROFILE_BRACKETS;
+static_assert(ZK_PROFILE_BRACKETS >= 0 && ZK_PROFILE_BRACKETS <= 2, "ZK_PROFILE_BRACKETS: 0 events, 1 nofence, 2 dispatch");
+
 struct Profiler {
     uint32_t mask = 0;
     struct Rec { int cls; hipEvent_t a, b; double bytes, ops; };
@@ -32,19 +41,33 @@
     hipEvent_t get() {
         if (!pool.empty()) { hipEvent_t e = pool.back(); pool.pop_back(); return e; }
         hipEvent_t e = nullptr;
-        (void)hipEventCreate(&e);
+        if (kBracketMode == BR_NOFENCE) (void)hipEventCreateWithFlags(&e, hipEventDisableSystemFence);
+        else (void)hipEventCreate(&e);
         return e;
     }
     bool on(int cls) const { return (mask >> cls) & 1u; }
 };
 
 struct ScopedKernelTimer {
-    Profiler* p; int cls; double bytes, ops; hipStream_t s; hipEvent_t a = nullptr;
-    ScopedKernelTimer(Profiler* p_, int cls_, double bytes_, hipStream_t s_, double ops_ = 0.0) : p(p_), cls(cls_), bytes(bytes_), ops(ops_), s(s_) {
-        if (p && p->on(cls)) { a = p->get(); (void)hipEventRecord(a, s); }
+    Profiler* p; int cls; double bytes, ops; hipStream_t s; hipEvent_t a = nullptr, b = nullptr; bool around = false;
+    ScopedKernelTimer(Profiler* p_, int cls_, double bytes_, hipStream_t s_, double ops_ = 0.0, bool span = false)
+        : p(p_ && p_->on(cls_) ? p_ : nullptr), cls(cls_), bytes(bytes_), ops(ops_), s(s_) {
+        if (p && (span || kBracketMode != BR_DISPATCH)) { around = true; a = p->get(); (void)hipEventRecord(a, s); }
+    }
+    ScopedKernelTimer(const ScopedKernelTimer&) = delete;
+    template <typename... P>
+    void launch(void (*kern)(P...), dim3 grid, dim3 block, size_t shmem, typename std::common_type<P>::type... args) {
+        if (p && !around && !a) {
+            a = p->get(); b = p->get();
+            void* argv[] = {(void*)&args...};
+            (void)hipExtLaunchKernel(reinterpret_cast<const void*>(kern), grid, block, argv, shmem, s, a, b, 0);
+        } else {
+            hipLaunchKernelGGL(kern, grid, block, shmem, s, args...);
+        }
     }
     ~ScopedKernelTimer() {
-        if (a) { hipEvent_t b = p->get(); (void)hipEventRecord(b, s); p->recs.push_back({cls, a, b, bytes, ops}); }
+        if (around) { b = p->get(); (void)hipEventRecord(b, s); }
+        if (a) p->recs.push_back({cls, a, b, bytes, ops});
     }
 };
 
@@ -110,6 +133,8 @@
 hipError_t launch_degree_check(const uint32_t* coef, uint32_t log_m, uint32_t nd, const uint32_t* dig_bits, uint32_t bound, uint32_t* out, hipStream_t s);
 
 hipError_t launch_build_inv_xm1(uint32_t* out, uint32_t logN, PowTable htab, uint32_t shift_mont, hipStream_t s);
+hipError_t launch_build_vz(uint32_t* out, uint32_t logN, uint32_t log_b, PowTable htab, uint32_t shift_mont, uint32_t gm1_mont, uint32_t gm2_mont,
+                           uint32_t gm3_mont, const uint32_t* zden, hipStream_t s);
 hipError_t launch_build_inv_xm1_range(uint32_t* out, size_t count, uint32_t e0, uint32_t log_order, PowTable htab, uint32_t shift_mont, hipStream_t s);
 hipError_t launch_halo_pack(const uint32_t* loc, uint32_t* out, uint32_t log_per, uint32_t lg, uint32_t h, hipStream_t s);
 hipError_t launch_interleave(const uint32_t* in, uint32_t* out, uint32_t log_parts, uint32_t log_cnt, hipStream_t s);
@@ -134,6 +159,8 @@
     uint32_t last;
     uint32_t alpha0_mont;
     uint32_t alpha1g2_mont;
+    uint32_t alpha2_mont;
+    const uint32_t* vz;
     uint32_t zz[32];
 };
 hipError_t launch_compose(const ComposeArgs& a, hipStream_t s, Profiler* prof = nullptr);
diff --git a/zkstark_amd/csrc/ntt_fast.hip b/zkstark_amd/csrc/ntt_fast.hip
--- a/zkstark_amd/csrc/ntt_fast.hip
+++ b/zkstark_amd/csrc/ntt_fast.hip
@@ -282,36 +282,36 @@
 }
 
 template <uint32_t MODE, int LA, int LB, int TILE_LOG>
-hipError_t launch3(const NttPassArgs& a, bool staged, uint32_t blocks, hipStream_t s) {
+hipError_t launch3(const NttPassArgs& a, bool staged, uint32_t blocks, ScopedKernelTimer& tm) {
     constexpr int R = 1 << (LA + LB), C = 1 << (TILE_LOG - LA - LB);
     size_t shmem = ((size_t)R * (C + 1) + R) * sizeof(uint32_t);
     const dim3 grid(blocks, a.batch ? a.batch : 1);
     if (MODE == NTT_DIT_LDE && a.prep) {
         if (a.logS >= 1) {
             shmem += (size_t)(C >> a.logS) * (R + 1) * sizeof(uint32_t);
-            hipLaunchKernelGGL((ntt_pass_fast_kernel<MODE, LA, LB, true, TILE_LOG, MODE == NTT_DIT_LDE ? 2 : 0>), grid, dim3(kThreads), shmem, s, a);
+            tm.launch((ntt_pass_fast_kernel<MODE, LA, LB, true, TILE_LOG, MODE == NTT_DIT_LDE ? 2 : 0>), grid, dim3(kThreads), shmem, a);
         } else {
-            hipLaunchKernelGGL((ntt_pass_fast_kernel<MODE, LA, LB, true, TILE_LOG, MODE == NTT_DIT_LDE ? 1 : 0>), grid, dim3(kThreads), shmem, s, a);
-        }
-    }
-    else if (staged) hipLaunchKernelGGL((ntt_pass_fast_kernel<MODE, LA, LB, true, TILE_LOG, 0>), grid, dim3(kThreads), shmem, s, a);
-    else hipLaunchKernelGGL((ntt_pass_fast_kernel<MODE, LA, LB, false, TILE_LOG, 0>), grid, dim3(kThreads), shmem, s, a);
+            tm.launch((ntt_pass_fast_kernel<MODE, LA, LB, true, TILE_LOG, MODE == NTT_DIT_LDE ? 1 : 0>), grid, dim3(kThreads), shmem, a);
+        }
+    }
+    else if (staged) tm.launch((ntt_pass_fast_kernel<MODE, LA, LB, true, TILE_LOG, 0>), grid, dim3(kThreads), shmem, a);
+    else tm.launch((ntt_pass_fast_kernel<MODE, LA, LB, false, TILE_LOG, 0>), grid, dim3(kThreads), shmem, a);
     return hipGetLastError();
 }
 
 template <uint32_t MODE, int LA, int LB>
-hipError_t launch2(const NttPassArgs& a, bool staged, uint32_t blocks, hipStream_t s) {
-    return a.tile_log == kSmallTileLog ? launch3<MODE, LA, LB, (int)kSmallTileLog>(a, staged, blocks, s)
-                                       : launch3<MODE, LA, LB, (int)kMidTileLog>(a, staged, blocks, s);
+hipError_t launch2(const NttPassArgs& a, bool staged, uint32_t blocks, ScopedKernelTimer& tm) {
+    return a.tile_log == kSmallTileLog ? launch3<MODE, LA, LB, (int)kSmallTileLog>(a, staged, blocks, tm)
+                                       : launch3<MODE, LA, LB, (int)kMidTileLog>(a, staged, blocks, tm);
 }
 
 template <uint32_t MODE>
-hipError_t launch1(const NttPassArgs& a, bool staged, uint32_t blocks, hipStream_t s) {
+hipError_t launch1(const NttPassArgs& a, bool staged, uint32_t blocks, ScopedKernelTimer& tm) {
     switch (a.logR) {
-        case 5: return launch2<MODE, 3, 2>(a, staged, blocks, s);
-        case 6: return launch2<MODE, 3, 3>(a, staged, blocks, s);
-        case 7: return launch2<MODE, 4, 3>(a, staged, blocks, s);
-        case 8: return launch2<MODE, 4, 4>(a, staged, blocks, s);
+        case 5: return launch2<MODE, 3, 2>(a, staged, blocks, tm);
+        case 6: return launch2<MODE, 3, 3>(a, staged, blocks, tm);
+        case 7: return launch2<MODE, 4, 3>(a, staged, blocks, tm);
+        case 8: return launch2<MODE, 4, 4>(a, staged, blocks, tm);
     }
     return hipErrorInvalidValue;
 }
@@ -327,14 +327,14 @@
     return true;
 }
 
-bool launch_ntt_pass_fast(const NttPassArgs& a, NttMode mode, hipStream_t s, hipError_t* err) {
+bool launch_ntt_pass_fast(const NttPassArgs& a, NttMode mode, ScopedKernelTimer& tm, hipError_t* err) {
     if (!ntt_fast_ok(a, mode)) return false;
     const bool staged = a.logS < a.tile_log - a.logR;
     const uint32_t blocks = 1u << (a.log_total - a.tile_log);
     switch (mode) {
-        case NTT_DIF: *err = launch1<NTT_DIF>(a, staged, blocks, s); break;
-        case NTT_DIT: *err = launch1<NTT_DIT>(a, staged, blocks, s); break;
-        case NTT_DIT_LDE: *err = launch1<NTT_DIT_LDE>(a, true, blocks, s); break;
+        case NTT_DIF: *err = launch1<NTT_DIF>(a, staged, blocks, tm); break;
+        case NTT_DIT: *err = launch1<NTT_DIT>(a, staged, blocks, tm); break;
+        case NTT_DIT_LDE: *err = launch1<NTT_DIT_LDE>(a, true, blocks, tm); break;
     }
     return true;
 }
diff --git a/zkstark_amd/csrc/zkstark.hip b/zkstark_amd/csrc/zkstark.hip
--- a/zkstark_amd/csrc/zkstark.hip
+++ b/zkstark_amd/csrc/zkstark.hip
@@ -106,6 +106,8 @@
 
 namespace {
 
+constexpr uint32_t kPendingProof = 0xffffffffu;
+
 template <typename T>
 int dmalloc(zk_ctx* c, T** p, size_t bytes) {
     hipError_t e = hipMalloc((void**)p, bytes ? bytes : 4);
@@ -503,7 +505,7 @@
             open_val(c, layer, leaf); open_path(c, layer, (size_t)1 << log_len, leaf);
         });
     if ((rc = open_launch(c))) return rc;
-    if ((rc = flush_host_parts(c))) return rc;
+    if (c->n_segs) { c->pending_top = true; c->pending_tree = kPendingProof; }
     lap("free term + fetch enqueue");
     if ((rc = open_wait(c))) return rc;
     lap("fetch wait");
@@ -965,6 +967,7 @@
     if (!c) return fail(ZK_ERR_INVALID, "null context");
     if (!c->have_trace) return fail(ZK_ERR_STATE, "zk_lde: no trace uploaded");
     HIPCHK(hipSetDevice(c->device));
+    if (int prc = settle_pending(c)) return prc;
     static const bool timing = getenv("ZK_HOST_TIMING") != nullptr;
     const double t0 = now_us();
     int rc = do_lde(c);
@@ -998,6 +1001,7 @@
     if (!c || !alpha_raw) return fail(ZK_ERR_INVALID, "zk_compose: null argument");
     if (!c->have_lde) return fail(ZK_ERR_STATE, "zk_compose: run zk_lde first");
     HIPCHK(hipSetDevice(c->device));
+    if (int prc = settle_pending(c)) return prc;
     return do_compose(c, alpha_raw);
 }
 
@@ -1005,6 +1009,7 @@
     if (!c) return fail(ZK_ERR_INVALID, "null context");
     if (round >= c->R) return fail(ZK_ERR_INVALID, "zk_fri_fold: round %u out of range (%u rounds)", round, c->R);
     HIPCHK(hipSetDevice(c->device));
+    if (int prc = settle_pending(c)) return prc;
     c->skipped_layers &= ~((uint64_t)1 << (2 + round));
     return do_fold(c, round, beta_raw);
 }
@@ -1013,6 +1018,7 @@
     if (steps < 1 || steps > kMaxFoldLog) return fail(ZK_ERR_INVALID, "zk_fri_fold_multi: steps must be 1..%u (got %u)", kMaxFoldLog, steps);
     if (round >= c->R || round + steps > c->R) return fail(ZK_ERR_INVALID, "zk_fri_fold_multi: rounds %u..%u out of range (%u rounds)", round, round + steps, c->R);
     HIPCHK(hipSetDevice(c->device));
+    if (int prc = settle_pending(c)) return prc;
     c->skipped_layers &= ~((uint64_t)1 << (1 + round + steps));
     return dom_fold_multi(c->dom, c->d_layers + c->layer_off[1 + round], c->d_layers + c->layer_off[1 + round + steps], c->L - round, round, steps,
                           beta_raw, c->stream, prof_of(c));
@@ -1035,6 +1041,7 @@
     for (size_t i = 0; i < count; ++i)
         if (in[i] >= P) return fail(ZK_ERR_INVALID, "zk_layer_write: value %zu is not a canonical residue", i);
     HIPCHK(hipSetDevice(c->device));
+    if (int prc = settle_pending(c)) return prc;
     HIPCHK(hipMemcpyAsync(c->d_layers + c->layer_off[layer] + offset, in, count * 4, hipMemcpyHostToDevice, c->stream));
     HIPCHK(hipStreamSynchronize(c->stream));
     if (layer == 0) c->have_lde = true;
```

New measurement: 2.929 billion. No clear change (-0.1%).
